# LudoMichaud/hlsjs-p2p-wrapper

Hardware: AMD Instinct MI355X
Metric: segments/sec + P2P offload ratio, 1080p 6 Mb/s HLS at 1/2/4/8 MI355X (higher is better)
Workload: dtype uint8

## Files before the change

hlsjs_p2p_wrapper_amd/agent/node.py:

```python
from __future__ import annotations

import contextlib
import logging
import os
import threading
import time
import zlib
from dataclasses import dataclass, field
from typing import Any, Dict, List, Optional, Tuple

import numpy as np
import torch

from ..net import http
from ..net.event_loop import get_event_loop
from ..ops import crc as _crc
from ..ops import segment as _seg
from ..ops._native import runtime as _rt
from ..parallel.comm import LocalComm, SwarmComm
from ..utils.trace import PhaseTimer, RequestTrace, TraceLog

log = logging.getLogger("hlsjs_p2p_wrapper_amd.node")

MAGIC = 0x48505032
HDR = 16
CHECK_WORD = 10
CDN_BOUND_BUSY = 0.6
ALIGN = 256
SLACK = 4096
PIN_DELAY_ROUNDS = 2


def swarm_id_for(content_id: str) -> int:
    return zlib.crc32(content_id.encode()) & 0x7FFFFFFF


_M32 = 0xFFFFFFFF


W_FORCE_CDN, W_NOT_STAGED, W_STAGING, W_PREFETCH, W_PY, W_CORRUPT = 1, 2, 4, 8, 16, 32
W_ON_DEV = 128
SRC_CDN, SRC_P2P, SRC_CACHE = 0, 1, 2
SOURCE_NAMES = ("cdn", "p2p", "cache")


class SwarmPeerLost(TimeoutError):
    """A swarm collective did not complete: a peer died, or stopped answering within the
    round / control deadline (``gpuSwarm.roundTimeoutMs`` / ``controlTimeoutMs``).  The
    message carries this rank's plan of the last round it posted."""


class Request:

    __slots__ = ("node", "key", "url", "headers", "callbacks", "agent", "aborted", "done", "t_submit", "token")

    def __init__(self, node: "SwarmNode", key: Tuple[int, int, int, int], url: str, headers: Dict[str, str],
                 callbacks: Any, agent: Any = None, aborted: bool = False, done: bool = False,
                 t_submit: float = 0.0) -> None:
        self.node = node
        self.key = key
        self.url = url
        self.headers = headers
        self.callbacks = callbacks
        self.agent = agent
        self.aborted = aborted
        self.done = done
        self.t_submit = t_submit
        self.token = None

    def abort(self) -> None:
        if not self.aborted:
            self.aborted = True
            if self.token is not None:
                self.node._abort_token(self.token)

    def __repr__(self) -> str:
        return f"Request(key={self.key}, url={self.url!r}, aborted={self.aborted}, done={self.done})"


class _WantX:

    __slots__ = ("url", "headers", "net", "src", "staged", "staging")

    def __init__(self, url: str, headers: Dict[str, str], net=None, src=None, staged: bool = True) -> None:
        self.url = url
        self.headers = headers
        self.net = net
        self.src = src
        self.staged = staged
        self.staging = False


@dataclass(eq=False)
class RoundHandle:
    round: int
    all_leaving: bool
    empty: bool = True
    ids: Any = None
    cdn: Any = None
    recv: Any = None
    failed: Any = None
    send_pins: Optional[np.ndarray] = None
    hold: List[np.ndarray] = field(default_factory=list)
    keep: List[Any] = field(default_factory=list)
    release: List[Any] = field(default_factory=list)
    sent_bytes: int = 0
    ev_cdn: Any = None
    dmas: int = 0
    ev_p2p: Any = None
    cdn_ms: float = 0.0
    p2p_ms: float = 0.0
    shaped_ms: float = 0.0
    ok_dev: Any = None
    ok_host: Any = None
    defer: Any = None
    expect_host: Any = None
    plan: Any = None
    t_post: float = 0.0
    done: Any = None
    n_wants: int = 0
    n_send: int = 0
    t0: float = 0.0
    completed: bool = False


class VerifyTicket:

    __slots__ = ("node", "eid", "expect", "token", "stamp", "done")

    def __init__(self, node: "SwarmNode", eid: int, expect: int, token: int) -> None:
        self.node = node
        self.eid = eid
        self.expect = expect
        self.token = token
        self.stamp = int(node._vround[eid])
        self.done = False

    def report(self, ok: bool) -> None:
        if not self.done:
            self.done = True
            node, e = self.node, self.eid
            if node._vflag[e] and node._vround[e] == self.stamp:
                node.verify_done(np.array([e], dtype=np.int64), np.array([bool(ok)]),
                                 np.array([self.token], dtype=np.int64))

    def __repr__(self) -> str:
        return f"VerifyTicket(eid={self.eid}, expect={self.expect:#010x}, done={self.done})"


class _EventPool:

    def __init__(self) -> None:
        self._free: Dict[bool, List[Any]] = {True: [], False: []}

    def get(self, timing: bool = False):
        free = self._free[timing]
        return free.pop() if free else torch.cuda.Event(enable_timing=timing)

    def put(self, timing: bool, *events) -> None:
        self._free[timing].extend(e for e in events if e is not None)


class SwarmNode:

    def __init__(self, comm: Optional[SwarmComm] = None, device: Any = "auto", cache_bytes: int = 1 << 30,
                 loop=None, cdn_dedup: bool = True, round_interval_ms: Optional[float] = None,
                 auto_tick: bool = True, max_wants_per_round: Optional[int] = None) -> None:
        self.comm = comm or LocalComm()
        self.rank = self.comm.rank
        self.world = self.comm.world_size
        self.ingest_crc = self.world > 1 or os.environ.get("HLSP2P_INGEST_CRC", "0") == "1"
        if device in (None, "auto"):
            device = torch.device("cuda", torch.cuda.current_device()) if torch.cuda.is_available() else "cpu"
        self.device = torch.device(device)
        self.is_cuda = self.device.type == "cuda"
        self.loop = loop or get_event_loop()
        self.rt = _rt()
        self.cache_bytes = int(cache_bytes)
        self.store = self.rt.SegmentStore(self.cache_bytes, ALIGN)
        self.directory = self.rt.Directory()
        self.arena = torch.empty(self.cache_bytes + SLACK, dtype=torch.uint8, device=self.device)
        self.stream = torch.cuda.Stream(self.device) if self.is_cuda else None
        self.copy_stream = (torch.cuda.Stream(self.device) if self.is_cuda and
                            os.environ.get("HLSP2P_COPY_STREAM", "1") != "0" else None)
        with self._on_node_stream():
            self.crc_dev = torch.zeros(self._crc_capacity(), dtype=torch.int32, device=self.device)
        self._events = _EventPool()
        self._clk = None
        self.online = True
        self._upload_default = True
        self._download_default = True
        self._sessions: Dict[Any, Tuple[bool, bool]] = {}
        self.cdn_dedup = cdn_dedup
        self.round = 0
        self.round_interval_ms = round_interval_ms
        self.round_timeout_s: Optional[float] = None
        self._last_posted: Optional[RoundHandle] = None
        self._exit_at = None
        fe = os.environ.get("HLSP2P_FAULT_EXIT")
        if fe:
            fr, _, fk = fe.partition(":")
            if int(fr) == self.rank:
                self._exit_at = int(fk)
        self.auto_tick = auto_tick
        self.max_wants_per_round = max_wants_per_round
        self.leaving = False
        self.closed = False
        self.failed: Optional[str] = None
        self.last_complete: Optional[float] = None
        self._wt = self.rt.WantTable()
        self._wx: Dict[int, _WantX] = {}
        self._tok_req: Dict[int, Request] = {}
        self._next_tok = -2
        self._bulk: Any = None
        self._bulk_hits: List[Tuple[np.ndarray, np.ndarray]] = []
        self._bulk_hits_scheduled = False
        self._locs: Dict[Tuple[str, Optional[str]], Tuple[int, int, int, int]] = {}
        self._locs_gen = -1
        self._loc_keep: Dict[int, torch.Tensor] = {}
        self._locator = self.rt.SegmentLocator()
        self._locator_gen = -1
        self._locator_origins: Dict[int, Any] = {}
        self._locator_skip: set = set()
        self._tick_scheduled = False
        self._timer = None
        self._pins: List[Tuple[int, np.ndarray]] = []
        self._inflight: Dict[int, RoundHandle] = {}
        self._local_hits: Dict[int, int] = {}
        self._delayed: Dict[int, Tuple[np.ndarray, np.ndarray]] = {}
        self._delayed_seq = 0
        self.pin_holders: List[Any] = []
        self.expect_holders: List[Any] = []
        self.audit_on = os.environ.get("HLSP2P_AUDIT", "0") == "1"
        self._agents: List[Any] = []
        self._prefetched: Dict[Tuple[int, int, int, int], str] = {}
        self._net_wants = False
        self.peer_online = np.ones(self.world, dtype=bool)
        self.stats = {"cdn": 0, "p2p": 0, "upload": 0, "cache": 0, "rounds": 0, "crc_failures": 0,
                      "segments": 0, "cdn_segments": 0, "p2p_segments": 0, "prefetched": 0,
                      "p2p_links": 0, "p2p_wire": 0, "p2p_rejected": 0, "p2p_rejected_segments": 0,
                      "cache_segments": 0}
        self.swarm_stats = {"cdn": 0, "p2p": 0, "upload": 0}
        self.last_round: Dict[str, Any] = {}
        self.corrupt_next_recv = 0
        self.misroute_next_send = 0
        self.divergence_check = self.world > 1 and os.environ.get("HLSP2P_DIVERGENCE_CHECK", "1") != "0"
        self._plan_digest = 0
        self._plan_round = 0
        self.p2p_from = np.zeros(self.world, dtype=np.int64)
        self.verify_deferred = False
        self.cdn_balance = os.environ.get("HLSP2P_CDN_BALANCE", "0") == "1"
        self._cdn_busy = 0.0
        self._cdn_num = self._cdn_den = 0.0
        self._cdn_t = None
        self._vflag = np.zeros(0, dtype=bool)
        self._vinfo = np.zeros((0, 10), dtype=np.int64)
        self._vround = np.zeros(0, dtype=np.int64)
        self._vexp = np.zeros(0, dtype=np.int64)
        self._vwait: Dict[int, List[np.ndarray]] = {}
        self.defer_inproc = False
        self._force_cdn_keys: set = set()
        self.link_kbps: Dict[int, float] = {}
        self.timer = PhaseTimer()
        self.trace: Optional[TraceLog] = None
        self.metrics_server: Any = None
        self._lock = threading.RLock()
        if self.world > 1 and auto_tick:
            self._timer = self.loop.set_interval(self._timer_tick, round_interval_ms or 10.0)

    def attach(self, agent: Any) -> None:
        self._agents.append(agent)

    def detach(self, agent: Any) -> None:
        if agent in self._agents:
            self._agents.remove(agent)
        self._sessions.pop(agent, None)
        gone = [t for t, r in self._tok_req.items() if r.agent is agent]
        for t in gone:
            self._tok_req.pop(t, None)
            self._wt.abort1(t)

    def set_session_flags(self, session: Any, download: bool, upload: bool) -> None:
        self._sessions[session] = (bool(download), bool(upload))

    def session_flags(self, session: Any) -> Tuple[bool, bool]:
        return self._sessions.get(session, (self._download_default, self._upload_default))

    @property
    def download_on(self) -> bool:
        if self._sessions:
            return any(d for d, _ in self._sessions.values())
        return self._download_default

    @download_on.setter
    def download_on(self, on: bool) -> None:
        self._download_default = bool(on)

    @property
    def upload_on(self) -> bool:
        if self._sessions:
            return any(u for _, u in self._sessions.values())
        return self._upload_default

    @upload_on.setter
    def upload_on(self, on: bool) -> None:
        self._upload_default = bool(on)

    @property
    def flags(self) -> int:
        f = 0
        if self.online:
            f |= self.rt.FLAG_ONLINE
        if self.upload_on:
            f |= self.rt.FLAG_UPLOAD
        if self.download_on:
            f |= self.rt.FLAG_DOWNLOAD
        if self.cdn_dedup:
            f |= self.rt.FLAG_CDN_DEDUP
        if self.cdn_balance and self._cdn_busy > CDN_BOUND_BUSY:
            f |= self.rt.FLAG_CDN_BOUND
        return f

    def pending(self) -> int:
        return len(self._wt)

    def _resolve(self, url: str, headers: Optional[Dict[str, str]]) -> Tuple[int, int, int, int, Optional[_WantX]]:
        rng_hdr = (headers.get("Range") or headers.get("range")) if headers else None
        gen = http.generation()
        if gen != self._locs_gen:
            self._locs.clear()
            self._locs_gen = gen
        ck = (url, rng_hdr)
        hit = self._locs.get(ck)
        if hit is not None:
            return hit[0], hit[1], hit[2], hit[3], None
        origin, path = http.resolve(url)
        if id(origin) not in self._locator_origins or self._locator_gen != http.generation():
            self._register_locator(origin)
        rng = http.parse_range(headers) if headers else None
        if getattr(origin, "staged_fetch", False):
            size = origin.staged_size(path, rng)
            self._net_wants = True
            x = _WantX(url, dict(headers or {}), net=(origin, path, rng), staged=size is not None)
            return int(size or 0), 0, 0, W_PY | (0 if size is not None else W_NOT_STAGED), x
        locate = getattr(origin, "locate", None)
        loc = locate(path, url, rng) if locate is not None else None
        if loc is None:
            size = origin.size(path, url, rng)
            return int(size or 0), 0, 0, W_PY, _WantX(url, dict(headers or {}), src=(origin, path, rng))
        data, off, n = loc
        base = data.data_ptr()
        flags = 0
        if data.is_cuda:
            flags |= W_ON_DEV
        elif base not in self._loc_keep and self.is_cuda and not data.is_pinned():
            raise RuntimeError("CDN origin buffers must be pinned host memory for the async H2D path")
        self._loc_keep.setdefault(base, data)
        corrupt = bool(getattr(origin, "_corrupt", None)) and origin.should_corrupt(path)
        if corrupt:
            flags |= W_CORRUPT
        res = (int(n), base + int(off), base, flags)
        if not corrupt and not getattr(origin, "_failures", None):
            if len(self._locs) > 1 << 16:
                self._locs.clear()
            self._locs[ck] = res
        return res[0], res[1], res[2], res[3], None

    def _register_locator(self, origin: Any) -> None:
        if http.generation() != self._locator_gen:
            self._locator.clear()
            self._locator_origins.clear()
            self._locator_skip.clear()
            self._locator_gen = http.generation()
        if id(origin) in self._locator_skip:
            return
        dirs_fn = getattr(origin, "segment_dirs", None)
        if dirs_fn is None:
            self._locator_skip.add(id(origin))
            return
        dirs = dirs_fn()
        if not dirs:
            return
        if any(not d[5].is_cuda and self.is_cuda and not d[5].is_pinned() for d in dirs):
            self._locator_skip.add(id(origin))
            return
        for d, prefix, suffix, lo, hi, data, offs, lens in dirs:
            base = data.data_ptr()
            self._loc_keep.setdefault(base, data)
            self._locator.add_dir(d, prefix, suffix, int(lo), int(hi), base, W_ON_DEV if data.is_cuda else 0,
                                  np.asarray(offs, dtype=np.int64), np.asarray(lens, dtype=np.int64))
        self._locator_origins[id(origin)] = origin

    def _locator_usable(self) -> bool:
        if not len(self._locator) or self._locator_gen != http.generation():
            return False
        for o in self._locator_origins.values():
            if getattr(o, "_failures", None) or getattr(o, "_corrupt", None):
                self._locator.clear()
                self._locator_origins.clear()
                return False
        return True

    def request(self, key: Tuple[int, int, int, int], url: str, headers: Optional[Dict[str, str]],
                callbacks: Any, agent: Any = None, view: Any = None) -> Request:
        k0, k1, k2, k3 = key
        k = (int(k0) & _M32, int(k1) & _M32, int(k2) & _M32, int(k3) & _M32)
        req = Request(self, k, url, dict(headers) if headers else {}, callbacks, agent, False, False,
                      self.loop.now())
        eid = self.store.lookup1(*k)
        if eid >= 0:
            self.store.pin(np.array([eid], dtype=np.int64))
            self._local_hits[eid] = self._local_hits.get(eid, 0) + 1
            self.loop.call_soon(self._serve_local, req, eid)
            return req
        if self._prefetched:
            self._prefetched.pop(k, None)
        wt = self._wt
        flags = 0
        if agent is not None and self._sessions and not self.session_flags(agent)[0]:
            flags = W_FORCE_CDN
        if self._force_cdn_keys and k in self._force_cdn_keys:
            self._force_cdn_keys.discard(k)
            flags |= W_FORCE_CDN
        size = ptr = base = 0
        x = None
        if wt.lookup1(*k) < 0:
            try:
                size, ptr, base, wf, x = self._resolve(url, req.headers)
            except http.HttpError as e:
                self.loop.call_soon(self._fail, req, e)
                return req
            flags |= wf
        tok = self._next_tok
        self._next_tok = tok - 1
        req.token = tok
        self._tok_req[tok] = req
        r = wt.add1(k[0], k[1], k[2], k[3], size, ptr, base, flags, tok)
        if r < 0 and x is not None:
            self._wx[-r - 1] = x
        self._schedule()
        return req

    def set_bulk_sink(self, sink: Any) -> None:
        self._bulk = sink

    def request_batch(self, keys: np.ndarray, urls: List[str], headers: Optional[List[Optional[Dict[str, str]]]],
                      tokens: np.ndarray, force_cdn: Optional[np.ndarray] = None) -> None:
        n = len(tokens)
        if n == 0:
            return
        keys = np.ascontiguousarray(np.asarray(keys, dtype=np.int64).reshape(n, 4) & _M32)
        tokens = np.ascontiguousarray(tokens, dtype=np.int64)
        eids = self.store.lookup(keys, False)
        hit = eids >= 0
        if hit.any():
            he = eids[hit]
            self.store.pin(he)
            self._bulk_hits.append((tokens[hit], he))
            if not self._bulk_hits_scheduled:
                self._bulk_hits_scheduled = True
                self.loop.call_soon(self._serve_bulk_hits)
            miss = np.flatnonzero(~hit)
            if not len(miss):
                return
        else:
            miss = None
        if self._vflag.any():
            miss = self._park_on_pending(keys, tokens, miss)
            if miss is not None and not len(miss):
                return
        idx = range(n) if miss is None else miss.tolist()
        m = n if miss is None else len(miss)
        sizes = np.zeros(m, dtype=np.int64)
        ptrs = np.zeros(m, dtype=np.int64)
        bases = np.zeros(m, dtype=np.int64)
        flags = np.zeros(m, dtype=np.int64)
        if force_cdn is not None:
            fc = np.asarray(force_cdn, dtype=bool)
            flags[:] = np.where(fc if miss is None else fc[miss], W_FORCE_CDN, 0)
        if self._force_cdn_keys:
            fk = self._force_cdn_keys
            for j, row in enumerate((keys if miss is None else keys[miss]).tolist()):
                t = tuple(row)
                if t in fk:
                    fk.discard(t)
                    flags[j] |= W_FORCE_CDN
        xs: Dict[int, _WantX] = {}
        bad: List[Tuple[int, int]] = []
        resolve = self._resolve
        done = None
        if self._locator_usable():
            sel_urls = urls if miss is None else [urls[i] for i in idx]
            s_, p_, b_, f_, done, found = self._locator.resolve(sel_urls if isinstance(sel_urls, list)
                                                                else list(sel_urls))
            if headers is not None:
                done &= np.fromiter((not h or ("Range" not in h and "range" not in h)
                                     for h in (headers if miss is None else [headers[i] for i in idx])),
                                    dtype=bool, count=m)
            sizes[done] = s_[done]
            ptrs[done] = p_[done]
            bases[done] = b_[done]
            flags[done] |= f_[done]
            if done.all():
                idx = ()
        for j, i in enumerate(idx):
            if done is not None and done[j]:
                continue
            try:
                sizes[j], ptrs[j], bases[j], wf, x = resolve(urls[i], headers[i] if headers is not None else None)
            except http.HttpError as e:
                bad.append((j, int(e.status or 0) or 500))
                continue
            flags[j] |= wf
            if x is not None:
                xs[j] = x
        sel_keys = keys if miss is None else keys[miss]
        sel_tok = tokens if miss is None else tokens[miss]
        if bad:
            bj = np.asarray([j for j, _ in bad], dtype=np.int64)
            self._fail_bulk(sel_tok[bj], np.asarray([s for _, s in bad], dtype=np.int64))
            keep = np.ones(m, dtype=bool)
            keep[bj] = False
            remap = np.cumsum(keep) - 1
            xs = {int(remap[j]): x for j, x in xs.items()}
            sel_keys, sel_tok = sel_keys[keep], sel_tok[keep]
            sizes, ptrs, bases, flags = sizes[keep], ptrs[keep], bases[keep], flags[keep]
        if self._prefetched:
            for kk in map(tuple, sel_keys.tolist()):
                self._prefetched.pop(kk, None)
        ids, created = self._wt.add(sel_keys, sizes, ptrs, bases, flags, sel_tok)
        for j, x in xs.items():
            if created[j]:
                self._wx[int(ids[j])] = x
        self._schedule()

    def abort_tokens(self, tokens: np.ndarray) -> int:
        return int(self._wt.abort(np.ascontiguousarray(tokens, dtype=np.int64)))

    def _abort_token(self, token: int) -> None:
        self._tok_req.pop(token, None)
        self._wt.abort1(token)

    def _stage(self, wid: int, x: _WantX) -> None:
        if x.staging or x.staged or x.net is None:
            return
        origin, path, rng = x.net
        x.staging = True
        self._wt.set(wid, -1, W_STAGING, 0)
        loop = self.loop
        loop.hold()

        def done(n, err):
            try:
                loop.call_soon_threadsafe(self._on_staged, wid, x, n, err)
            finally:
                loop.release()

        origin.stage(path, x.url, rng, x.headers, done)

    def _on_staged(self, wid: int, x: _WantX, n, err) -> None:
        x.staging = False
        alive = self._wx.get(wid) is x
        if err is not None:
            if alive:
                self._finish_failed(np.array([wid], dtype=np.int64), err)
            return
        x.staged = True
        if alive and self._wt.set(wid, int(n), 0, W_STAGING | W_NOT_STAGED):
            self._schedule()
        else:
            origin, path, rng = x.net
            origin.release(path, rng)

    def prefetch(self, key: Tuple[int, int, int, int], url: str, headers: Optional[Dict[str, str]] = None) -> bool:
        k = tuple(int(v) & _M32 for v in key)
        if self._wt.lookup1(*k) >= 0 or self.store.lookup1(*k) >= 0:
            return False
        try:
            size, ptr, base, wf, x = self._resolve(url, dict(headers or {}))
        except http.HttpError:
            return False
        r = self._wt.add1(k[0], k[1], k[2], k[3], size, ptr, base, wf | W_PREFETCH, self.rt.NO_TOKEN)
        if r < 0 and x is not None:
            self._wx[-r - 1] = x
        self.stats["prefetched"] += 1
        self._schedule()
        return True

    def _schedule(self) -> None:
        if self.world == 1 and self.auto_tick and not self._tick_scheduled:
            self._tick_scheduled = True
            self.loop.call_soon(self._local_tick)

    def _local_tick(self) -> None:
        self._tick_scheduled = False
        if len(self._wt):
            self.tick()

    def _timer_tick(self) -> None:
        if not self.closed:
            self.tick()

    def _serve_local(self, req: Request, eid: int) -> None:
        try:
            if req.aborted:
                return
            off, n = (int(x) for x in self.store.entries(np.array([eid], dtype=np.int64))[0][:2])
            src = self._prefetched.pop(req.key, None)
            if src is None:
                self.stats["cache"] += n
                self.stats["cache_segments"] += 1
            self._deliver_req(req, src or "cache", n, 0.0, 0.0, self.arena[off:off + n], -1, eid)
        finally:
            self.store.unpin(np.array([eid], dtype=np.int64))
            n = self._local_hits.get(eid, 0) - 1
            if n > 0:
                self._local_hits[eid] = n
            else:
                self._local_hits.pop(eid, None)

    def _park_on_pending(self, keys: np.ndarray, tokens: np.ndarray, miss: Optional[np.ndarray]) -> np.ndarray:
        rows = np.arange(len(tokens)) if miss is None else miss
        pe = self.store.lookup(np.ascontiguousarray(keys[rows]), True)
        park = pe >= 0
        park[park] = pe[park] < len(self._vflag)
        park[park] = self._vflag[pe[park]]
        if not park.any():
            return rows if miss is not None else None
        for e, t in zip(pe[park].tolist(), tokens[rows[park]].tolist()):
            self._vwait.setdefault(e, []).append(t)
        self.stats["parked"] = self.stats.get("parked", 0) + int(park.sum())
        return rows[~park]

    def _release_parked(self, e: int, ok: bool) -> None:
        toks = np.asarray(self._vwait.pop(e), dtype=np.int64)
        if ok:
            arr = np.array([e], dtype=np.int64)
            ids = np.repeat(arr, len(toks))
            self.store.pin(ids)
            self._bulk_hits.append((toks, ids))
            if not self._bulk_hits_scheduled:
                self._bulk_hits_scheduled = True
                self.loop.call_soon(self._serve_bulk_hits)
        else:
            self._retry_cdn(self._vinfo[e], toks)

    def _serve_bulk_hits(self) -> None:
        self._bulk_hits_scheduled = False
        hits, self._bulk_hits = self._bulk_hits, []
        for tok, eids in hits:
            try:
                ent = self.store.entries(eids)
                offs, lens = ent[:, 0].copy(), ent[:, 1].copy()
                self.stats["cache"] += int(lens.sum())
                self.stats["cache_segments"] += len(tok)
                z = np.zeros(len(tok), dtype=np.float64)
                self._deliver_cols(tok, np.full(len(tok), SRC_CACHE, dtype=np.int8), lens, z, z, offs, eids)
            finally:
                self.store.unpin(eids)

    def _fail(self, req: Request, err: Exception) -> None:
        if req.aborted or req.done:
            return
        req.done = True
        cb = req.callbacks
        on_error = cb.get("onError") if isinstance(cb, dict) else getattr(cb, "onError", None)
        if on_error is not None:
            on_error(err)

    def _fail_bulk(self, tokens: np.ndarray, status: np.ndarray) -> None:
        if self._bulk is not None and len(tokens):
            self._bulk.fail(tokens, status)

    def _finish_failed(self, wids: np.ndarray, err: http.HttpError) -> None:
        tok, _, _ = self._wt.finish(np.ascontiguousarray(wids, dtype=np.int64))
        for w in wids.tolist():
            x = self._wx.pop(w, None)
            if x is not None and x.net is not None and x.staged:
                x.net[0].release(x.net[1], x.net[2])
        if not len(tok):
            return
        bulk = tok >= 0
        if bulk.any():
            self._fail_bulk(tok[bulk], np.full(int(bulk.sum()), int(err.status or 0) or 500, dtype=np.int64))
        for t in tok[~bulk].tolist():
            req = self._tok_req.pop(t, None)
            if req is not None:
                self.loop.call_soon(self._fail, req, err)

    def _encode(self, rows: np.ndarray, adds: np.ndarray, rms: np.ndarray) -> np.ndarray:
        hdr = np.zeros(HDR, dtype=np.int64)
        hdr[0] = MAGIC
        hdr[1] = self.flags
        hdr[2] = len(rows)
        hdr[3] = len(adds)
        hdr[4] = len(rms)
        hdr[5] = 1 if self.leaving else 0
        hdr[6] = self.round
        hdr[7] = self.stats["cdn"]
        hdr[8] = self.stats["p2p"]
        hdr[9] = self.stats["upload"]
        hdr[CHECK_WORD] = self.directory.digest
        hdr[CHECK_WORD + 1] = self._plan_digest
        hdr[CHECK_WORD + 2] = self._plan_round
        return np.concatenate([hdr, rows.reshape(-1), adds.reshape(-1).astype(np.int64),
                               rms.reshape(-1).astype(np.int64)])

    CRC_TABLE_MAX = 1 << 20

    def _crc_capacity(self) -> int:
        return int(min(max(1024, self.cache_bytes // (8 << 10) + 1), self.CRC_TABLE_MAX))

    def _on_node_stream(self):
        return torch.cuda.stream(self.stream) if self.stream is not None else contextlib.nullcontext()

    def _grow_crc(self, n: int) -> None:
        old = self.crc_dev
        if n <= old.numel():
            return
        with self._on_node_stream():
            new = torch.zeros(max(n, 2 * old.numel()), dtype=torch.int32, device=self.device)
            new[:old.numel()] = old
        if old.is_cuda:
            old.record_stream(self.stream)
        self.crc_dev = new

    def tick(self) -> bool:
        with self._lock:
            h = self.launch_round()
            self.complete_round(h)
            return h.all_leaving

    def launch_round(self) -> RoundHandle:
        h = self._launch_round()
        if self.audit_on:
            from .audit import audit_node

            audit_node(self, "launch_round")
        return h

    def complete_round(self, h: RoundHandle) -> None:
        self._complete_round(h)
        if self.audit_on:
            from .audit import audit_node

            audit_node(self, "complete_round")

    def _launch_round(self) -> RoundHandle:
        rt = self.rt
        t0 = time.perf_counter()
        self.round += 1
        self.stats["rounds"] += 1
        if self._exit_at is not None and self.round >= self._exit_at:
            log.error("rank %d: injected crash at round %d (HLSP2P_FAULT_EXIT)", self.rank, self.round)
            os._exit(17)
        if self.verify_deferred and self.round % 8 == 0 and len(self._vflag):
            self._sweep_pending()
        if self._pins:
            keep = []
            for rel, ids in self._pins:
                if rel <= self.round:
                    self.store.unpin(ids)
                else:
                    keep.append((rel, ids))
            self._pins = keep
        for agent in self._agents:
            hook = getattr(agent, "before_round", None)
            if hook is not None:
                hook()
        cap = self.max_wants_per_round
        ids, rows, dropped, too_big, deferred = self._wt.select(self.store, self.directory,
                                                               -1 if cap is None else int(cap), self.round)
        if len(dropped) and self._wx:
            for w in dropped.tolist():
                x = self._wx.pop(w, None)
                if x is not None and x.net is not None and x.staged:
                    x.net[0].release(x.net[1], x.net[2])
        if len(too_big):
            self._finish_failed(too_big, http.HttpError(507, "", f"segment exceeds the {self.cache_bytes}-byte cache"))
        if deferred:
            self.stats["deferred"] = self.stats.get("deferred", 0) + int(deferred)
        if len(rows):
            need = int(np.maximum((rows[:, 4] + (ALIGN - 1)) // ALIGN * ALIGN, ALIGN).sum())
            self.store.retire_region(need)
            if not self.store.wrap_for(need):
                raise RuntimeError("segment cache cannot wrap for the round (pinned entries block eviction)")
            if self.audit_on:
                from .audit import check_region

                check_region(self, need)
        adds, rms = self.store.take_delta()
        try:
            parts = self.comm.allgather_control(self._encode(rows, adds, rms))
        except Exception as e:
            raise self._peer_lost("control all-gather", e) from e
        try:
            all_wants, flags, all_leaving, swarm_tot = rt.ingest_control(
                self.directory, parts, MAGIC, HDR, CHECK_WORD if self.divergence_check else -1)
        except rt.SwarmDivergence as e:
            self._diverged(str(e))
            raise
        self.peer_online = (flags & rt.FLAG_ONLINE) != 0
        self.swarm_stats = {"cdn": int(swarm_tot[0]), "p2p": int(swarm_tot[1]), "upload": int(swarm_tot[2])}
        h = RoundHandle(self.round, all_leaving, t0=t0)
        h.ids = ids
        self._inflight[h.round] = h
        t_ctrl = time.perf_counter()
        self.timer.add("control", t_ctrl - t0)
        if not len(all_wants):
            self._plan_digest, self._plan_round = 0, self.round
            return h
        h.empty = False
        me = self.rank
        cdn_bytes = np.fromiter((int(p[7]) for p in parts), dtype=np.int64, count=len(parts)) \
            if self.cdn_balance and self.world > 1 else None
        plan, any_p2p, self._plan_digest = rt.plan_round_for(self.directory, all_wants, flags, self.world, me,
                                                             cdn_bytes)
        self._plan_round = self.round
        h.n_wants = len(all_wants)
        cdn_rows = plan[(plan[:, 5] == -1) & (plan[:, 6] == me)]
        if self._net_wants and self._wx:
            for wid in plan[(plan[:, 5] == -2) & (plan[:, 6] == me), 7].tolist():
                x = self._wx.get(wid)
                if x is not None:
                    self._stage(wid, x)
        send_rows = plan[plan[:, 5] == me]
        recv_rows = plan[(plan[:, 6] == me) & (plan[:, 5] >= 0)]
        h.n_send = len(send_rows)
        h.plan = (send_rows, recv_rows)
        self._last_posted = h
        send_eids = np.full(len(send_rows), -1, dtype=np.int64)
        cached = send_rows[:, 8] == 0
        if cached.any():
            eids = self.store.lookup(np.ascontiguousarray(send_rows[cached, :4]), False)
            send_eids[cached] = eids
            valid = eids[eids >= 0]
            if len(valid):
                self.store.pin(valid)
                h.send_pins = valid
            if self.misroute_next_send > 0:
                self._misroute(send_rows, send_eids)
        t_cdn0 = time.perf_counter()
        self.timer.add("plan", t_cdn0 - t_ctrl)
        with (torch.cuda.stream(self.stream) if self.is_cuda else contextlib.nullcontext()):
            if len(cdn_rows):
                self._cdn_phase(h, cdn_rows)
                seeded = np.flatnonzero(~cached)
                if len(seeded) and h.cdn is not None:
                    send_eids[seeded] = self.store.lookup(np.ascontiguousarray(send_rows[seeded, :4]), False)
            t_p2p0 = time.perf_counter()
            self.timer.add("cdn_enqueue", t_p2p0 - t_cdn0)
            if any_p2p:
                self._p2p_phase(h, send_rows, recv_rows, send_eids)
            h.sent_bytes = int(send_rows[:, 4].sum()) if len(send_rows) else 0
            if self.is_cuda:
                h.done = self._events.get(True)
                h.done.record(self.stream)
        self.timer.add("p2p_enqueue", time.perf_counter() - t_p2p0)
        return h

    def _complete_round(self, h: RoundHandle) -> None:
        if h.completed:
            return
        h.completed = True
        self._inflight.pop(h.round, None)
        if h.empty:
            self.last_complete = time.monotonic()
            self.last_round = {"wants": 0, "ms": (time.perf_counter() - h.t0) * 1e3}
            if h.ids is not None and len(h.ids):
                self._wt.requeue(h.ids, False)
            return
        t0 = time.perf_counter()
        if h.done is not None and not h.done.query():
            self._wait_round(h)
            self._clock_sync(h.done, time.perf_counter())
            h.done = None
        t1 = time.perf_counter()
        self.timer.add("wait_device", t1 - t0)
        if h.ev_cdn is not None:
            h.cdn_ms = h.ev_cdn[0].elapsed_time(h.ev_cdn[1])
            self._events.put(True, *h.ev_cdn)
        if h.ev_p2p is not None:
            h.p2p_ms = h.ev_p2p[0].elapsed_time(h.ev_p2p[1])
            if self._clk is not None:
                ev, t_host = self._clk
                q = t_host + ev.elapsed_time(h.ev_p2p[0]) / 1e3 - h.t_post
                self.timer.add("exchange_queued", max(0.0, q))
                self.timer.add("exchange_queued_n", 1.0)
            self._events.put(True, *h.ev_p2p)
        if h.done is not None:
            self._events.put(True, h.done)
            h.done = None
        wt = self._wt
        recv = h.recv
        good = bad = None
        dgood = exp_good = None
        if recv is not None:
            ok = (h.ok_host.numpy() if isinstance(h.ok_host, torch.Tensor) else np.asarray(h.ok_host)).astype(bool)
            if ok.all():
                good = recv
            else:
                good = tuple(c[ok] for c in recv)
                bad = tuple(c[~ok] for c in recv)
            if h.defer is not None:
                dgood = h.defer[ok]
                eh = h.expect_host.numpy() if isinstance(h.expect_host, torch.Tensor) else np.asarray(h.expect_host)
                eh = eh.astype(np.int32) ^ _crc.key_digest(recv[5])
                exp_good = eh.astype(np.int64)[ok]
                if not dgood.any():
                    dgood = None
            commit = good[2] if dgood is None else good[2][~dgood]
            if len(commit):
                self.store.commit(commit)
            self._count_p2p(good[4], True)
            if bad is not None:
                self.store.drop(bad[2])
                self.stats["crc_failures"] += len(bad[0])
                self._count_p2p(bad[4], False)
        if h.send_pins is not None:
            self.store.unpin(h.send_pins)
        for x in h.release:
            origin, path, rng = x.net
            origin.release(path, rng)
        self.stats["upload"] += h.sent_bytes
        t2 = time.perf_counter()
        if h.cdn is not None and len(h.cdn[0]):
            wids, eids, offs, lens = h.cdn[0], h.cdn[1], h.cdn[2], h.cdn[3]
            self.stats["cdn"] += int(lens.sum())
            self.stats["cdn_segments"] += len(wids)
            tok, idx, pf = wt.finish(wids)
            self._after_finish(wids, pf, h.cdn[4], "cdn")
            cdn_ms = max(h.cdn_ms, h.shaped_ms)
            k = len(tok)
            if k:
                self._deliver_cols(tok, np.zeros(k, dtype=np.int8), lens[idx], np.full(k, cdn_ms),
                                   np.zeros(k), offs[idx], eids[idx], delay=h.shaped_ms)
        if good is not None and len(good[0]):
            wids, srcs, eids, offs, lens, keys = good
            winfo = wt.info(np.ascontiguousarray(wids[dgood])) if dgood is not None else None
            tok, idx, pf = wt.finish(wids)
            exp_tok = None
            if dgood is not None:
                tok, idx, exp_tok = self._settle_deferred(h, good, dgood, exp_good, tok, idx, winfo)
            self._after_finish(wids, pf, keys, "p2p")
            k = len(tok)
            if k:
                p2p_ms = np.full(len(wids), h.p2p_ms)
                delay = None
                if self.link_kbps:
                    delay = np.zeros(len(wids))
                    link_q: Dict[int, int] = {}
                    for i, (src, n) in enumerate(zip(srcs.tolist(), lens.tolist())):
                        kbps = self.link_kbps.get(src)
                        if kbps:
                            link_q[src] = link_q.get(src, 0) + n
                            delay[i] = link_q[src] * 8.0 / kbps
                            p2p_ms[i] = max(p2p_ms[i], delay[i])
                    delay = delay[idx]
                self._deliver_cols(tok, np.ones(k, dtype=np.int8), lens[idx], np.zeros(k), p2p_ms[idx], offs[idx],
                                   eids[idx], peers=srcs[idx], delay=delay, expect=exp_tok)
        if bad is not None and len(bad[0]):
            wt.requeue(bad[0], True)
        if h.ids is not None and len(h.ids):
            served = [a for a in (h.cdn[0] if h.cdn is not None else None,
                                  h.recv[0] if h.recv is not None else None, h.failed) if a is not None and len(a)]
            rest = np.setdiff1d(h.ids, np.concatenate(served), assume_unique=False) if served else h.ids
            if len(rest):
                wt.requeue(rest, False)
        for ids in h.hold:
            self.store.unpin(ids)
        h.hold = []
        self.timer.add("commit", t2 - t1)
        self.timer.add("deliver", time.perf_counter() - t2)
        self.timer.add("dev_cdn_ms", h.cdn_ms / 1e3)
        now = time.perf_counter()
        if self._cdn_t is not None:
            self._cdn_num += 0.2 * (h.cdn_ms / 1e3 - self._cdn_num)
            self._cdn_den += 0.2 * ((now - self._cdn_t) - self._cdn_den)
            self._cdn_busy = min(1.0, self._cdn_num / self._cdn_den) if self._cdn_den > 0 else 0.0
        self._cdn_t = now
        self.timer.add("dev_p2p_ms", h.p2p_ms / 1e3)
        self.last_complete = time.monotonic()
        self.last_round = {"wants": h.n_wants, "cdn": 0 if h.cdn is None else len(h.cdn[0]), "send": h.n_send,
                           "recv": 0 if h.recv is None else len(h.recv[0]), "cdn_ms": h.cdn_ms, "dmas": h.dmas,
                           "p2p_ms": h.p2p_ms, "ms": (time.perf_counter() - h.t0) * 1e3}
        if wt.waiting:
            self._schedule()

    def _after_finish(self, wids: np.ndarray, prefetch_only: np.ndarray, keys: np.ndarray, source: str) -> None:
        if self._wx:
            for w in wids.tolist():
                x = self._wx.pop(w, None)
                if x is not None and x.net is not None and x.staged and source == "p2p":
                    x.net[0].release(x.net[1], x.net[2])
        if prefetch_only.any():
            for i in np.flatnonzero(prefetch_only).tolist():
                self._prefetched[tuple(int(v) for v in keys[i])] = source

    def _clock_sync(self, ev, t_host: float) -> None:
        old = self._clk
        self._clk = (ev, t_host)
        if old is not None:
            self._events.put(True, old[0])

    ROUND_SPIN_S = 0.02

    def _wait_round(self, h: RoundHandle) -> None:
        ev = h.done
        spin_end = time.perf_counter() + self.ROUND_SPIN_S
        while time.perf_counter() < spin_end:
            if ev.query():
                return
        check = getattr(self.comm, "async_error", None)
        deadline = time.perf_counter() + self.round_deadline_s()
        while not ev.query():
            err = check() if check is not None else ""
            if err:
                self.failed = self.failed or f"round {h.round}: data plane error: {err}"
                raise RuntimeError(f"rank {self.rank}: swarm round {h.round} failed in the data plane: {err}")
            if time.perf_counter() > deadline:
                summary = self.plan_summary(h)
                log.error("rank %d: swarm round %d did not complete; this rank's plan: %s", self.rank, h.round,
                          summary)
                self._dump_plan(h)
                self.failed = self.failed or f"round {h.round} did not complete within {self.round_deadline_s():g} s"
                raise SwarmPeerLost(f"rank {self.rank}: swarm round {h.round} did not complete on the device "
                                    f"within {self.round_deadline_s():g} s (gpuSwarm.roundTimeoutMs); a peer may have "
                                    f"stopped.  Plan: {summary}")
            time.sleep(1e-3)

    ROUND_TIMEOUT_S = 60.0

    def round_deadline_s(self) -> float:
        if self.round_timeout_s is not None:
            return float(self.round_timeout_s)
        return float(os.environ.get("HLSP2P_ROUND_TIMEOUT", str(self.ROUND_TIMEOUT_S)))

    def _peer_lost(self, where: str, err: BaseException) -> "SwarmPeerLost":
        summary = self.plan_summary(self._last_posted) if self._last_posted is not None else {}
        log.error("rank %d: swarm %s failed in round %d: %s; last posted plan: %s", self.rank, where, self.round,
                  err, summary)
        self._diverged(f"{where} failed: {err}")
        return SwarmPeerLost(f"rank {self.rank}: swarm {where} failed in round {self.round} ({type(err).__name__}: "
                             f"{err}); a peer may have stopped.  Plan of round "
                             f"{summary.get('round', '-')}: {summary}")

    @staticmethod
    def plan_summary(h: RoundHandle) -> Dict[str, Any]:
        out: Dict[str, Any] = {"round": h.round, "send": {}, "recv": {}}
        if h.plan is None:
            return out
        for name, rows, col in (("send", h.plan[0], 6), ("recv", h.plan[1], 5)):
            if len(rows):
                peers, inv = np.unique(rows[:, col], return_inverse=True)
                nbytes = np.bincount(inv, weights=rows[:, 4])
                count = np.bincount(inv)
                out[name] = {int(p): [int(c), int(b)] for p, c, b in zip(peers, count, nbytes)}
        return out

    def _dump_plan(self, h: RoundHandle) -> None:
        d = os.environ.get("HLSP2P_PLAN_DUMP")
        if not d or h.plan is None:
            return
        try:
            os.makedirs(d, exist_ok=True)
            np.savez(os.path.join(d, f"plan.r{h.round}.rank{self.rank}.npz"), send=h.plan[0], recv=h.plan[1],
                     directory_digest=np.int64(self.directory.digest))
        except OSError as e:
            log.warning("rank %d: plan dump failed: %s", self.rank, e)

    def _diverged(self, what: str) -> None:
        if self.failed is None:
            self.failed = what
        log.error("rank %d: %s", self.rank, what)
        abort = getattr(self.comm, "abort", None)
        if abort is not None:
            try:
                abort()
            except Exception as e:
                log.warning("rank %d: communicator abort failed: %s", self.rank, e)

    def _views(self, offs: List[int], lens: List[int]) -> List[torch.Tensor]:
        if not len(offs):
            return []
        if self.is_cuda:
            from ..ops._native import device as _dev

            return _dev().arena_views(self.arena, np.asarray(offs, dtype=np.int64), np.asarray(lens, dtype=np.int64))
        arena = self.arena
        return [arena[o:o + n] for o, n in zip(offs, lens)]

    def _cdn_phase(self, h: RoundHandle, cdn_rows: np.ndarray) -> None:
        wids = np.ascontiguousarray(cdn_rows[:, 7])
        info = self._wt.info(wids)
        ptrs = info[:, 5].copy()
        bases = info[:, 6].copy()
        lens = info[:, 4].copy()
        wflags = info[:, 7]
        keep = info[:, 0] >= 0
        failed: List[int] = []
        slow = np.flatnonzero(keep & ((wflags & W_PY) != 0))
        for i in slow.tolist():
            wid = int(wids[i])
            x = self._wx.get(wid)
            try:
                if x is None:
                    raise http.HttpError(500, "", "want lost its origin state")
                if x.net is not None:
                    origin, path, rng = x.net
                    data, off, n, _ = origin.resource_range(path, rng)
                    h.release.append(x)
                    self._wx.pop(wid, None)
                    x.staged = False
                else:
                    origin, path, rng = x.src
                    data, off, n, _ = origin.resource(path)
                    if rng is not None:
                        s, e = rng
                        e = n - 1 if e is None else min(e, n - 1)
                        off, n = off + s, max(0, e - s + 1)
                    if origin.should_corrupt(path):
                        wflags[i] |= W_CORRUPT
            except http.HttpError as e:
                self._finish_failed(np.array([wid], dtype=np.int64), e)
                failed.append(wid)
                keep[i] = False
                continue
            base = data.data_ptr()
            if not data.is_cuda and self.is_cuda and base not in self._loc_keep and not data.is_pinned():
                raise RuntimeError("CDN origin buffers must be pinned host memory for the async H2D path")
            if data.is_cuda:
                wflags[i] |= W_ON_DEV
            h.keep.append(data)
            ptrs[i], bases[i], lens[i] = base + int(off), base, int(n)
        if failed:
            h.failed = np.asarray(failed, dtype=np.int64)
        if not keep.all():
            wids, ptrs, bases, lens, wflags = wids[keep], ptrs[keep], bases[keep], lens[keep], wflags[keep]
            keys = np.ascontiguousarray(info[keep, :4])
        else:
            keys = np.ascontiguousarray(info[:, :4])
        if not len(wids):
            return
        res = self.store.reserve_run(keys, lens, self.round)
        if res is None:
            raise RuntimeError("segment cache cannot make room (pinned entries block eviction)")
        _, eids, offs = res
        self.store.pin(eids)
        h.hold.append(eids)
        self._grow_crc(int(eids.max()) + 1)
        if self.is_cuda:
            on_dev = (wflags & W_ON_DEV) != 0
            if on_dev.any() and not on_dev.all():
                raise RuntimeError("CDN origin buffers of one round must all be pinned host or all HBM")
            start = self._events.get(True)
            end = self._events.get(True)
            cs = self.copy_stream
            with (torch.cuda.stream(cs) if cs is not None else contextlib.nullcontext()):
                start.record(cs if cs is not None else self.stream)
                from ..ops._native import device as _dev

                h.dmas = _dev().h2d_batch(self.arena, offs, ptrs, lens, bases, ALIGN, bool(on_dev[0]))
                end.record(cs if cs is not None else self.stream)
            if cs is not None:
                self.stream.wait_event(end)
            h.ev_cdn = (start, end)
        else:
            t = time.perf_counter()
            self.rt.host_copy_batch(self.arena.data_ptr(), self.arena.numel(), offs, ptrs, lens)
            h.cdn_ms = (time.perf_counter() - t) * 1e3
        corrupt = np.flatnonzero((wflags & W_CORRUPT) != 0)
        for i in corrupt.tolist():
            if lens[i]:
                self.arena[int(offs[i]) + int(lens[i]) // 2] ^= 0xFF
        if self.ingest_crc:
            _crc.crc32_batch(self.arena, offs, lens, scatter_to=self.crc_dev, scatter_idx=eids, keys=keys)
        self.store.commit(eids)
        total = int(lens.sum())
        h.shaped_ms = http.Shaper.transfer_ms(total)
        h.cdn = (wids, eids, offs, lens, keys)

    def _p2p_phase(self, h: RoundHandle, send_rows: np.ndarray, recv_rows: np.ndarray,
                   send_eids: np.ndarray) -> None:
        sends: List[Tuple[int, torch.Tensor]] = []
        recvs: List[Tuple[int, torch.Tensor]] = []
        dev = self.device
        t_prep = time.perf_counter()
        srun, gath, rrun, rid_a, roff_a = self.store.p2p_layout(
            np.ascontiguousarray(send_rows), np.ascontiguousarray(send_eids, dtype=np.int64),
            np.ascontiguousarray(recv_rows), self.round)
        spans_plane = getattr(self.comm, "exchange_spans", None) if self.is_cuda else None
        if spans_plane is not None and len(srun) and not (srun[:, 3] == 0).all():
            spans_plane = None
        trailer_all = trailers = None
        if len(send_rows):
            present_all = send_eids >= 0
            idx = _dev_index(np.where(present_all, send_eids, 0), dev)
            trailer_all = torch.index_select(self.crc_dev, 0, idx)
            if not present_all.all():
                trailer_all[torch.from_numpy(np.flatnonzero(~present_all)).to(dev)] = -1
            spans = self._views(srun[:, 4].tolist(), srun[:, 5].tolist()) \
                if spans_plane is None and len(srun) and (srun[:, 3] == 0).all() else None
            for k, (dst, a, b, mode, off, total) in enumerate(srun.tolist() if spans_plane is None else ()):
                if mode == 0:
                    buf = spans[k] if spans is not None else self.arena[off:off + total]
                else:
                    buf = torch.zeros(total, dtype=torch.uint8, device=dev)
                    g = gath[gath[:, 0] == k]
                    if len(g):
                        _seg.copy_segments(self.arena, buf, g[:, 1], g[:, 2], g[:, 3])
                sends.append((dst, buf))
                sends.append((dst, trailer_all[a:b]))
        if len(rrun):
            trailers = torch.empty(len(recv_rows), dtype=torch.int32, device=dev)
            if spans_plane is None:
                views = self._views(rrun[:, 3].tolist(), rrun[:, 4].tolist())
                for (src, a, b, _, _), view in zip(rrun.tolist(), views):
                    recvs.append((src, view))
                    recvs.append((src, trailers[a:b]))
            h.hold.append(rid_a)
            np.add.at(self.p2p_from, rrun[:, 0], np.add.reduceat(recv_rows[:, 4], rrun[:, 1]))
            self._grow_crc(int(rid_a.max()) + 1)
            h.recv = (np.ascontiguousarray(recv_rows[:, 7]), np.ascontiguousarray(recv_rows[:, 5]), rid_a, roff_a,
                      np.ascontiguousarray(recv_rows[:, 4]), np.ascontiguousarray(recv_rows[:, :4]))
        self.timer.add("p2p_prep", time.perf_counter() - t_prep)
        t = time.perf_counter()
        h.t_post = t
        if self.is_cuda:
            start = self._events.get(True)
            end = self._events.get(True)
            start.record(self.stream)
        try:
            if spans_plane is not None:
                spans_plane(*_span_columns(self.arena.data_ptr(), srun, trailer_all, rrun, trailers))
            else:
                self.comm.exchange(sends, recvs)
        except Exception as e:
            raise self._peer_lost("data-plane exchange", e) from e
        if self.is_cuda:
            end.record(self.stream)
            h.ev_p2p = (start, end)
        else:
            h.p2p_ms = (time.perf_counter() - t) * 1e3
        if h.recv is None:
            return
        if self.corrupt_next_recv > 0:
            self.corrupt_next_recv -= 1
            o, n = int(roff_a[0]), int(recv_rows[0, 4])
            if n:
                self.arena[o + n // 2] ^= 0x5A
        defer = None
        if self.verify_deferred:
            wf = self._wt.info(np.ascontiguousarray(recv_rows[:, 7]))[:, 7]
            d = (wf & (W_PY | W_PREFETCH)) == 0
            defer = d if d.any() else None
        if defer is None:
            _, ok = _crc.crc32_batch(self.arena, roff_a, recv_rows[:, 4], expect_dev=trailers,
                                     scatter_to=self.crc_dev, scatter_idx=rid_a, keys=recv_rows[:, :4])
        else:
            ok = self._defer_verify(h, defer, trailers, roff_a, recv_rows, rid_a)
        if isinstance(ok, np.ndarray):
            h.ok_host = ok
        elif self.is_cuda:
            h.ok_host = torch.empty(ok.numel(), dtype=torch.uint8, pin_memory=True)
            h.ok_host.copy_(ok, non_blocking=True)
        else:
            h.ok_host = ok
        self.stats["p2p_wire"] += int(recv_rows[:, 4].sum())
        self.stats["p2p_links"] += len(rrun)

    def _defer_verify(self, h: RoundHandle, defer: np.ndarray, trailers, roff_a: np.ndarray, recv_rows: np.ndarray,
                      rid_a: np.ndarray):
        dev = self.device
        nd, dd = np.flatnonzero(~defer), np.flatnonzero(defer)
        h.defer = defer
        if not len(nd):
            self.crc_dev.index_copy_(0, _dev_index(rid_a, dev), trailers)
            self._expect_to_host(h, trailers)
            return np.ones(len(recv_rows), dtype=np.uint8)
        if self.is_cuda:
            from ..ops.desc import pack_to_device

            ix = pack_to_device({"nd": nd, "dd": dd, "rd": np.ascontiguousarray(rid_a[dd])}, dev)
        else:
            ix = {"nd": torch.from_numpy(nd), "dd": torch.from_numpy(dd), "rd": torch.from_numpy(rid_a[dd])}
        ok = torch.ones(len(recv_rows), dtype=torch.uint8, device=dev)
        if len(nd):
            _, ok_nd = _crc.crc32_batch(self.arena, roff_a[nd], recv_rows[nd, 4],
                                        expect_dev=torch.index_select(trailers, 0, ix["nd"]),
                                        scatter_to=self.crc_dev, scatter_idx=rid_a[nd], keys=recv_rows[nd, :4])
            ok.index_copy_(0, ix["nd"], ok_nd)
        if len(dd):
            self.crc_dev.index_copy_(0, ix["rd"], torch.index_select(trailers, 0, ix["dd"]))
        self._expect_to_host(h, trailers)
        return ok

    def _expect_to_host(self, h: RoundHandle, trailers) -> None:
        if self.is_cuda:
            h.expect_host = torch.empty(trailers.numel(), dtype=torch.int32, pin_memory=True)
            h.expect_host.copy_(trailers, non_blocking=True)
        else:
            h.expect_host = trailers.clone()

    def _settle_deferred(self, h: RoundHandle, good: tuple, dgood: np.ndarray, exp_good: np.ndarray,
                         tok: np.ndarray, idx: np.ndarray, winfo: np.ndarray):
        wids, _, eids, offs, lens, _ = good
        n = len(wids)
        info = np.zeros((n, winfo.shape[1]), dtype=winfo.dtype)
        info[dgood] = winfo
        now = dgood & (np.bincount(idx, minlength=n) == 0)
        neg = tok < 0
        if neg.any() and not self.defer_inproc:
            now |= dgood & (np.bincount(idx[neg], minlength=n) > 0)
        keep = None
        if now.any():
            nr = np.flatnonzero(now)
            exp = (exp_good[nr] & _M32).tolist()
            if self.is_cuda:
                with self._on_node_stream():
                    _, okd = _crc.crc32_batch(self.arena, offs[nr], lens[nr], expect=exp)
                    ok_now = okd.cpu().numpy().astype(bool)
            else:
                ok_now = _crc.crc32_batch(self.arena, offs[nr], lens[nr], expect=exp)[1].numpy().astype(bool)
            if ok_now.any():
                self.store.commit(eids[nr[ok_now]])
            bad = nr[~ok_now]
            if len(bad):
                self.store.drop(eids[bad])
                self.stats["crc_failures"] += len(bad)
                self._reject_p2p(lens[bad])
                keep = np.ones(len(tok), dtype=bool)
                for r in bad.tolist():
                    sel = idx == r
                    self._retry_cdn(info[r], tok[sel])
                    keep &= ~sel
            dgood = dgood & ~now
        pend = np.flatnonzero(dgood)
        if len(pend):
            pe = eids[pend]
            self.store.pin(pe)
            self._vpend_add(pe, info[pend], exp_good[pend])
        exp_row = np.full(n, -1, dtype=np.int64)
        exp_row[pend] = exp_good[pend] & _M32
        if keep is not None:
            tok, idx = tok[keep], idx[keep]
        return tok, idx, exp_row[idx]

    def _misroute(self, send_rows: np.ndarray, send_eids: np.ndarray) -> None:
        ids, keys = self.store.resident()
        if not len(ids):
            return
        lens = self.store.entries(ids)[:, 1]
        for i in np.flatnonzero(send_eids >= 0).tolist():
            same = np.flatnonzero((lens == send_rows[i, 4]) & (keys != send_rows[i, :4]).any(axis=1))
            if len(same):
                send_eids[i] = ids[same[0]]
                self.misroute_next_send -= 1
                return

    def _count_p2p(self, lens: np.ndarray, passed: bool) -> None:
        n = len(lens)
        if not n:
            return
        b = int(np.asarray(lens, dtype=np.int64).sum())
        if passed:
            self.stats["p2p"] += b
            self.stats["p2p_segments"] += n
        else:
            self.stats["p2p_rejected"] += b
            self.stats["p2p_rejected_segments"] += n

    def _reject_p2p(self, lens: np.ndarray) -> None:
        n = len(lens)
        if not n:
            return
        b = int(np.asarray(lens, dtype=np.int64).sum())
        self.stats["p2p"] -= b
        self.stats["p2p_segments"] -= n
        self.stats["p2p_rejected"] += b
        self.stats["p2p_rejected_segments"] += n

    def _vpend_add(self, eids: np.ndarray, info: np.ndarray, expect: np.ndarray) -> None:
        need = int(eids.max()) + 1
        if need > len(self._vflag):
            cap = max(need, 2 * len(self._vflag), 1024)
            flag = np.zeros(cap, dtype=bool)
            flag[:len(self._vflag)] = self._vflag
            vinfo = np.zeros((cap, self._vinfo.shape[1]), dtype=np.int64)
            vinfo[:len(self._vinfo)] = self._vinfo
            vround = np.zeros(cap, dtype=np.int64)
            vround[:len(self._vround)] = self._vround
            vexp = np.zeros(cap, dtype=np.int64)
            vexp[:len(self._vexp)] = self._vexp
            self._vflag, self._vinfo, self._vround, self._vexp = flag, vinfo, vround, vexp
        self._vflag[eids] = True
        self._vinfo[eids] = info
        self._vround[eids] = self.round
        self._vexp[eids] = expect

    VERIFY_STALE_ROUNDS = 32

    def _sweep_pending(self) -> int:
        stale = np.flatnonzero(self._vflag & (self._vround < self.round - self.VERIFY_STALE_ROUNDS))
        if not len(stale):
            return 0
        ent = self.store.entries(stale)
        offs, lens = ent[:, 0].copy(), ent[:, 1].copy()
        exp = (self._vexp[stale] & _M32).tolist()
        if self.is_cuda:
            with self._on_node_stream():
                _, okd = _crc.crc32_batch(self.arena, offs, lens, expect=exp)
                ok = okd.cpu().numpy().astype(bool)
        else:
            ok = _crc.crc32_batch(self.arena, offs, lens, expect=exp)[1].numpy().astype(bool)
        self.verify_done(stale, ok, np.full(len(stale), self.rt.NO_TOKEN, dtype=np.int64))
        self.stats["verify_swept"] = self.stats.get("verify_swept", 0) + len(stale)
        return len(stale)

    def pending_verify(self) -> int:
        return int(self._vflag.sum())

    def _retry_cdn(self, info: np.ndarray, tokens: np.ndarray) -> None:
        tokens = np.ascontiguousarray(tokens, dtype=np.int64)
        if not len(tokens):
            return
        n = len(tokens)
        rep = np.repeat(info.reshape(1, -1), n, axis=0)
        self._wt.add(np.ascontiguousarray(rep[:, :4]), np.ascontiguousarray(rep[:, 4]), np.ascontiguousarray(rep[:, 5]),
                     np.ascontiguousarray(rep[:, 6]), np.ascontiguousarray(rep[:, 7] | W_FORCE_CDN), tokens)
        self._schedule()

    def invalidate(self, keys) -> int:
        keys = np.ascontiguousarray(np.asarray(keys, dtype=np.int64).reshape(-1, 4) & _M32)
        if not len(keys):
            return 0
        eids = self.store.lookup(keys, False)
        held = eids[eids >= 0]
        if len(held):
            self.store.detach(held)
        for row in keys.tolist():
            self._force_cdn_keys.add(tuple(row))
        self.stats["invalidated"] = self.stats.get("invalidated", 0) + len(held)
        return len(held)

    def verify_done(self, eids: np.ndarray, ok: np.ndarray, tokens: np.ndarray) -> int:
        eids = np.asarray(eids, dtype=np.int64)
        ok = np.asarray(ok, dtype=bool)
        tokens = np.asarray(tokens, dtype=np.int64)
        if not len(eids):
            return 0
        ue, inv = np.unique(eids, return_inverse=True)
        uok = np.ones(len(ue), dtype=bool)
        np.logical_and.at(uok, inv, ok)
        inside = ue < len(self._vflag)
        pend = np.zeros(len(ue), dtype=bool)
        pend[inside] = self._vflag[ue[inside]]
        good = ue[pend & uok]
        if len(good):
            self._vflag[good] = False
            self.store.commit(good)
            self.store.unpin(good)
            if self._vwait:
                for e in good.tolist():
                    if e in self._vwait:
                        self._release_parked(e, True)
        bad = np.flatnonzero(pend & ~uok)
        for k in bad.tolist():
            e = int(ue[k])
            self._vflag[e] = False
            arr = np.array([e], dtype=np.int64)
            self.store.detach(arr)
            self.store.unpin(arr)
            self.stats["crc_failures"] += 1
            self._reject_p2p(self._vinfo[e:e + 1, 4])
            toks = tokens[inv == k]
            self._retry_cdn(self._vinfo[e], toks[toks >= 0])
            if e in self._vwait:
                self._release_parked(e, False)
            if (toks <= -2).any():
                self._force_cdn_keys.add(tuple(int(v) & _M32 for v in self._vinfo[e][:4]))
        return len(bad)

    def _deliver_cols(self, tok: np.ndarray, src: np.ndarray, nbytes: np.ndarray, cdn_ms: np.ndarray,
                      p2p_ms: np.ndarray, offs: np.ndarray, eids: np.ndarray, peers: Optional[np.ndarray] = None,
                      delay: Any = None, expect: Optional[np.ndarray] = None) -> None:
        if delay is not None and not (np.isscalar(delay) and delay <= 0):
            d = np.broadcast_to(np.asarray(delay, dtype=np.float64), tok.shape)
            later = d > 0
            if later.any():
                li = np.flatnonzero(later)
                le = eids[li]
                le = le[le >= 0]
                if len(le):
                    self.store.pin(le)
                self._delayed_seq += 1
                self._delayed[self._delayed_seq] = (le, tok[li])
                self.loop.set_timeout(self._deliver_deferred, float(d[li].max()),
                                      (tok[li], src[li], nbytes[li], cdn_ms[li], p2p_ms[li], offs[li], eids[li],
                                       None if peers is None else peers[li], None,
                                       None if expect is None else expect[li]), le, self._delayed_seq)
                if later.all():
                    return
                ni = np.flatnonzero(~later)
                tok, src, nbytes, cdn_ms, p2p_ms, offs, eids = (tok[ni], src[ni], nbytes[ni], cdn_ms[ni], p2p_ms[ni],
                                                                offs[ni], eids[ni])
                peers = None if peers is None else peers[ni]
                expect = None if expect is None else expect[ni]
        pin = eids[eids >= 0]
        if len(pin):
            self.store.pin(pin)
            self._pins.append((self.round + PIN_DELAY_ROUNDS, pin))
        bulk = tok >= 0
        nb = int(bulk.sum())
        if nb:
            self.stats["segments"] += nb
            if self._bulk is not None:
                ex = {} if expect is None else {"expect": expect if nb == len(tok) else expect[bulk]}
                if nb == len(tok):
                    self._bulk.deliver(tok, src, nbytes, cdn_ms, p2p_ms, offs, eids, **ex)
                else:
                    self._bulk.deliver(tok[bulk], src[bulk], nbytes[bulk], cdn_ms[bulk], p2p_ms[bulk], offs[bulk],
                                       eids[bulk], **ex)
        if nb == len(tok):
            return
        obj = np.flatnonzero(~bulk)
        reqs = [self._tok_req.pop(t, None) for t in tok[obj].tolist()]
        live = [i for i, r in zip(obj.tolist(), reqs) if r is not None]
        if not live:
            return
        views = self._views(offs[live].tolist(), nbytes[live].tolist())
        for i, r, view in zip(live, [r for r in reqs if r is not None], views):
            if expect is not None and expect[i] >= 0:
                view.swarm_verify = VerifyTicket(self, int(eids[i]), int(expect[i]), r.token)
            self._deliver_req(r, SOURCE_NAMES[int(src[i])], int(nbytes[i]), float(cdn_ms[i]), float(p2p_ms[i]), view,
                              self.rank if peers is None else int(peers[i]), int(eids[i]), pin=False)

    def _deliver_deferred(self, cols, ids: np.ndarray, seq: int = 0) -> None:
        self._delayed.pop(seq, None)
        try:
            self._deliver_cols(*cols)
        finally:
            if len(ids):
                self.store.unpin(ids)

    def _deliver_req(self, req: Request, source: str, nbytes: int, cdn_ms: float, p2p_ms: float, data: Any,
                     peer: int, eid: int, pin: bool = True) -> None:
        if req.aborted or req.done:
            return
        if pin and eid >= 0:
            arr = np.array([eid], dtype=np.int64)
            self.store.pin(arr)
            self._pins.append((self.round + PIN_DELAY_ROUNDS, arr))
        req.done = True
        self.stats["segments"] += 1
        trace = self.trace
        if trace is not None:
            now = self.loop.now()
            xfer = p2p_ms if source == "p2p" else cdn_ms
            trace.add(RequestTrace(req.key, req.t_submit, max(req.t_submit, now - xfer), now, source, nbytes,
                                   peer if source == "p2p" else self.rank, self.round))
        if req.agent is not None:
            req.agent._account(source, nbytes)
        cb = req.callbacks
        if isinstance(cb, dict):
            on_progress, on_success = cb.get("onProgress"), cb.get("onSuccess")
        else:
            delivered = getattr(cb, "onDelivered", None)
            if delivered is not None:
                delivered(source, nbytes, cdn_ms, p2p_ms, data)
                return
            on_progress, on_success = getattr(cb, "onProgress", None), getattr(cb, "onSuccess", None)
        if on_progress is not None:
            p2p = source in ("p2p", "cache")
            on_progress({"cdnDownloaded": 0 if p2p else nbytes, "p2pDownloaded": nbytes if p2p else 0,
                         "cdnDuration": 0.0 if p2p else cdn_ms, "p2pDuration": p2p_ms if p2p else 0.0})
        if req.aborted:
            return
        if on_success is not None:
            on_success(data)

    def enable_trace(self, maxlen: int = 100_000) -> TraceLog:
        if self.trace is None:
            self.trace = TraceLog(maxlen)
        return self.trace

    def save_cache(self, path: str) -> Dict[str, int]:
        from .checkpoint import save_cache

        return save_cache(self, path)

    def load_cache(self, path: str) -> Dict[str, int]:
        from .checkpoint import load_cache

        return load_cache(self, path)

    def set_link_bandwidth(self, peer: int, kbps: Optional[float]) -> None:
        if kbps:
            self.link_kbps[int(peer)] = float(kbps)
        else:
            self.link_kbps.pop(int(peer), None)

    def set_online(self, online: bool) -> None:
        self.online = bool(online)

    def close(self, timeout_rounds: int = 100000) -> None:
        self.leaving = True
        if self._timer is not None:
            self._timer.cancel()
            self._timer = None
        try:
            if self.world > 1:
                for _ in range(timeout_rounds):
                    if self.tick():
                        break
        finally:
            self.closed = True
            if self.metrics_server is not None:
                srv, self.metrics_server = self.metrics_server, None
                srv.close()

    def swarm_offload_ratio(self) -> float:
        c, p = self.swarm_stats["cdn"], self.swarm_stats["p2p"]
        return p / (p + c) if (p + c) else 0.0


def _span_columns(arena_ptr: int, srun: np.ndarray, trailer_all, rrun: np.ndarray, trailers):
    def cols(runs, span_off, span_len, tr):
        n = len(runs)
        ptr = np.empty(2 * n, dtype=np.int64)
        nb = np.empty(2 * n, dtype=np.int64)
        peer = np.empty(2 * n, dtype=np.int64)
        if n:
            ptr[0::2] = arena_ptr + runs[:, span_off]
            nb[0::2] = runs[:, span_len]
            ptr[1::2] = tr.data_ptr() + 4 * runs[:, 1]
            nb[1::2] = 4 * (runs[:, 2] - runs[:, 1])
            peer[0::2] = peer[1::2] = runs[:, 0]
        return ptr, nb, peer

    sp, sb, sd = cols(srun, 4, 5, trailer_all)
    rp, rb, rs = cols(rrun, 3, 4, trailers)
    return sp, sb, sd, rp, rb, rs


def _dev_index(idx: np.ndarray, dev: torch.device) -> torch.Tensor:
    if dev.type == "cuda":
        from ..ops.desc import pack_to_device

        return pack_to_device({"i": np.ascontiguousarray(idx, dtype=np.int64)}, dev)["i"]
    return torch.from_numpy(np.ascontiguousarray(idx, dtype=np.int64))


_local = threading.local()


def current_node() -> Optional[SwarmNode]:
    return getattr(_local, "node", None)


def set_current_node(node: Optional[SwarmNode]) -> None:
    _local.node = node


def node_for_config(p2p_config: Any) -> SwarmNode:
    apply_network_config(p2p_config)
    node = current_node()
    if node is not None and not node.closed:
        return node
    cfg = {}
    if isinstance(p2p_config, dict):
        cfg = dict(p2p_config.get("gpuSwarm") or {})
    backend = cfg.get("backend", "auto")
    comm: SwarmComm
    if backend == "auto":
        import torch.distributed as dist

        backend = "dist" if (dist.is_available() and dist.is_initialized() and dist.get_world_size() > 1) else "local"
    if backend == "local":
        comm = LocalComm()
    elif backend == "thread":
        comm = cfg["hub"].comm(int(cfg["rank"]))
    elif backend == "dist":
        from ..parallel.comm import DistComm

        comm = DistComm()
    elif backend == "remote":
        from ..parallel.fleet import RemoteNode

        node = RemoteNode(cfg["conn"], world=int(cfg.get("world", 1)), rank=int(cfg.get("rank", 0)),
                          payload=bool(cfg.get("fleetPayload", False)))
        set_current_node(node)
        return node
    else:
        raise ValueError(f"unknown gpuSwarm backend {backend!r}")
    node = SwarmNode(comm, device=cfg.get("device", "auto"), cache_bytes=int(cfg.get("cacheBytes", 1 << 30)),
                     cdn_dedup=bool(cfg.get("cdnDedup", True)), round_interval_ms=cfg.get("roundIntervalMs"),
                     auto_tick=bool(cfg.get("autoTick", True)), max_wants_per_round=cfg.get("maxWantsPerRound"))
    if cfg.get("numaBind") and node.is_cuda:
        from ..utils.runtime import bind_to_gpu_numa

        bind_to_gpu_numa(node.device.index if node.device.index is not None else torch.cuda.current_device())
    if cfg.get("audit"):
        node.audit_on = True
    if cfg.get("roundTimeoutMs") is not None:
        node.round_timeout_s = float(cfg["roundTimeoutMs"]) / 1e3
    if cfg.get("controlTimeoutMs") is not None and hasattr(comm, "control_timeout_s"):
        comm.control_timeout_s = float(cfg["controlTimeoutMs"]) / 1e3
    if cfg.get("deferVerify"):
        node.verify_deferred = node.defer_inproc = True
    if cfg.get("trace"):
        node.enable_trace()
    for peer, kbps in (cfg.get("linkKbps") or {}).items():
        node.set_link_bandwidth(int(peer), kbps)
    if cfg.get("metricsPort") is not None:
        node.metrics_server = _start_metrics(node, cfg, backend)
    set_current_node(node)
    return node


def apply_network_config(p2p_config: Any) -> None:
    gs = p2p_config.get("gpuSwarm") if isinstance(p2p_config, dict) else None
    net = gs.get("network") if isinstance(gs, dict) else None
    if net and not http.network_enabled():
        http.enable_network(True, **(net if isinstance(net, dict) else {}))


def _start_metrics(node: SwarmNode, cfg: dict, backend: str) -> Any:
    from ..utils.metrics import MetricsServer

    port = int(cfg["metricsPort"])
    if port:
        local = os.environ.get("LOCAL_RANK") if backend == "dist" else None
        port += int(local) if local is not None else node.rank
    try:
        return MetricsServer(node, port=port, host=str(cfg.get("metricsHost", "127.0.0.1")))
    except OSError as e:
        log.warning("metrics endpoint disabled on rank %d: cannot bind port %d (%s)", node.rank, port, e)
        return None
```

hlsjs_p2p_wrapper_amd/ops/csrc/kernels/bindings.cpp:

```cpp
#include <c10/hip/HIPStream.h>
#include <hip/hip_runtime_api.h>
#include <torch/extension.h>
#include <pybind11/numpy.h>
#include <pybind11/stl.h>

#include <cstring>

namespace hlsp2p {
namespace dev {
int aes_chunk_blocks();
hipError_t launch_aes128_cbc_decrypt(const uint8_t*, uint8_t*, const int64_t*, const int64_t*, const int64_t*,
                                     const int64_t*, const uint32_t*, const uint32_t*, const uint32_t*,
                                     const uint8_t*, int64_t*, int, int64_t, int, hipStream_t, const int64_t*,
                                     const void*, uint32_t*, const int64_t*, void*);
hipError_t launch_crc32_batch(const uint8_t*, const int64_t*, const int64_t*, const int64_t*, const int64_t*,
                              const void*, const uint32_t*, uint32_t*, uint32_t*, const uint32_t*, uint8_t*,
                              const int64_t*, uint32_t*, int64_t, int, int64_t, int, bool, hipStream_t,
                              const int64_t*);
hipError_t launch_ts_demux(const uint8_t*, const int64_t*, const int64_t*, const int64_t*, int, int64_t, uint32_t*,
                           int64_t*, int32_t*, uint8_t*, const int64_t*, int64_t*, int64_t, int64_t*, hipStream_t,
                           const void*, const int64_t*);
hipError_t launch_segment_copy(const uint8_t*, uint8_t*, const int64_t*, const int64_t*, const int64_t*,
                               const int64_t*, int, int64_t, hipStream_t);
}
}

namespace {

using torch::Tensor;
namespace D = hlsp2p::dev;

void check(const Tensor& t, const char* name, c10::ScalarType dt, int64_t min_numel = 0) {
  TORCH_CHECK(t.is_cuda(), name, " must be a GPU tensor");
  TORCH_CHECK(t.is_contiguous(), name, " must be contiguous");
  TORCH_CHECK(t.scalar_type() == dt, name, " has dtype ", t.scalar_type(), ", expected ", dt);
  TORCH_CHECK(t.numel() >= min_numel, name, " too small: ", t.numel(), " < ", min_numel);
}

void same_device(const Tensor& a, const Tensor& b) {
  TORCH_CHECK(a.device() == b.device(), "tensors on different devices");
}

hipStream_t stream() { return c10::hip::getCurrentHIPStream().stream(); }

void ok(hipError_t e, const char* what) {
  TORCH_CHECK(e == hipSuccess, what, " launch failed: ", hipGetErrorString(e));
}

int num_cus(const Tensor& t) {
  static int cached[64] = {0};
  const int dev = t.get_device();
  if (dev >= 0 && dev < 64 && cached[dev]) return cached[dev];
  int n = 0;
  hipDeviceGetAttribute(&n, hipDeviceAttributeMultiprocessorCount, dev);
  if (n <= 0) n = 256;
  if (dev >= 0 && dev < 64) cached[dev] = n;
  return n;
}

template <typename T>
const T* cptr(const Tensor& t) { return reinterpret_cast<const T*>(t.data_ptr()); }
template <typename T>
T* mptr(const Tensor& t) { return reinterpret_cast<T*>(t.data_ptr()); }

void aes128_cbc_decrypt(Tensor src, Tensor dst, Tensor src_off, Tensor dst_off, Tensor blk_prefix,
                        Tensor chunk_prefix, Tensor drk, Tensor iv, Tensor td0, Tensor isb, Tensor out_len,
                        int64_t total_chunks) {
  const int64_t B = src_off.numel();
  check(src, "src", torch::kUInt8);
  check(dst, "dst", torch::kUInt8);
  check(src_off, "src_off", torch::kInt64);
  check(dst_off, "dst_off", torch::kInt64, B);
  check(blk_prefix, "blk_prefix", torch::kInt64, B + 1);
  check(chunk_prefix, "chunk_prefix", torch::kInt64, B + 1);
  check(drk, "drk", torch::kInt32, B * 44);
  check(iv, "iv", torch::kUInt8, B * 16);
  check(td0, "td0", torch::kInt32, 256);
  check(isb, "isb", torch::kUInt8, 256);
  check(out_len, "out_len", torch::kInt64, B);
  TORCH_CHECK(src.data_ptr() != dst.data_ptr(), "CBC decrypt cannot run in place");
  TORCH_CHECK((reinterpret_cast<uintptr_t>(src.data_ptr()) & 15) == 0 &&
                  (reinterpret_cast<uintptr_t>(dst.data_ptr()) & 15) == 0,
              "src/dst must be 16-byte aligned");
  same_device(src, dst);
  ok(D::launch_aes128_cbc_decrypt(cptr<uint8_t>(src), mptr<uint8_t>(dst), cptr<int64_t>(src_off),
                                  cptr<int64_t>(dst_off), cptr<int64_t>(blk_prefix), cptr<int64_t>(chunk_prefix),
                                  cptr<uint32_t>(drk), cptr<uint32_t>(iv), cptr<uint32_t>(td0), cptr<uint8_t>(isb),
                                  mptr<int64_t>(out_len), static_cast<int>(B), total_chunks, num_cus(src), stream(),
                                  nullptr, nullptr, nullptr, nullptr, nullptr),
     "aes128_cbc_decrypt");
}

void crc32_batch(Tensor buf, Tensor seg_off, Tensor seg_len, Tensor tile_prefix, Tensor res_off, Tensor wfrag,
                 Tensor tables, Tensor residues, Tensor crc_out, c10::optional<Tensor> expect,
                 c10::optional<Tensor> ok_out, int64_t total_tiles, c10::optional<Tensor> scatter_idx,
                 c10::optional<Tensor> scatter_out) {
  const int64_t B = seg_off.numel();
  check(buf, "buf", torch::kUInt8);
  check(seg_off, "seg_off", torch::kInt64);
  check(seg_len, "seg_len", torch::kInt64, B);
  check(tile_prefix, "tile_prefix", torch::kInt64, B + 1);
  check(res_off, "res_off", torch::kInt64, B);
  const bool fp4 = wfrag.scalar_type() == torch::kUInt8;
  check(wfrag, "wfrag", fp4 ? torch::kUInt8 : torch::kInt8, fp4 ? 32 * 64 * 16 : 64 * 64 * 16);
  check(tables, "tables", torch::kInt32, 48 * 1024);
  check(residues, "residues", torch::kInt32);
  check(crc_out, "crc_out", torch::kInt32, B);
  TORCH_CHECK((reinterpret_cast<uintptr_t>(buf.data_ptr()) & 15) == 0, "buf must be 16-byte aligned");
  const uint32_t* ex = nullptr;
  uint8_t* okp = nullptr;
  if (expect.has_value()) {
    check(*expect, "expect", torch::kInt32, B);
    ex = cptr<uint32_t>(*expect);
  }
  if (ok_out.has_value()) {
    check(*ok_out, "ok_out", torch::kUInt8, B);
    okp = mptr<uint8_t>(*ok_out);
  }
  const int64_t* sidx = nullptr;
  uint32_t* sout = nullptr;
  int64_t sn = 0;
  TORCH_CHECK(scatter_idx.has_value() == scatter_out.has_value(), "scatter_idx and scatter_out go together");
  if (scatter_out.has_value()) {
    check(*scatter_idx, "scatter_idx", torch::kInt64, B);
    check(*scatter_out, "scatter_out", torch::kInt32);
    sidx = cptr<int64_t>(*scatter_idx);
    sout = mptr<uint32_t>(*scatter_out);
    sn = scatter_out->numel();
  }
  ok(D::launch_crc32_batch(cptr<uint8_t>(buf), cptr<int64_t>(seg_off), cptr<int64_t>(seg_len),
                           cptr<int64_t>(tile_prefix), cptr<int64_t>(res_off), wfrag.data_ptr(),
                           cptr<uint32_t>(tables), mptr<uint32_t>(residues), mptr<uint32_t>(crc_out), ex, okp,
                           sidx, sout, sn, static_cast<int>(B), total_tiles, num_cus(buf), fp4, stream(), nullptr),
     "crc32_batch");
}

void ts_demux(Tensor buf, Tensor seg_off, Tensor seg_len, Tensor blk_prefix, int64_t total_blocks, Tensor meta,
              Tensor pts_dts, Tensor blk_sums, Tensor es, Tensor es_off, Tensor pes, int64_t max_pes, Tensor info) {
  const int64_t B = seg_off.numel();
  check(buf, "buf", torch::kUInt8);
  check(seg_off, "seg_off", torch::kInt64);
  check(seg_len, "seg_len", torch::kInt64, B);
  check(blk_prefix, "blk_prefix", torch::kInt64, B + 1);
  check(meta, "meta", torch::kInt32, total_blocks * 256);
  check(pts_dts, "pts_dts", torch::kInt64, total_blocks * 256 * 2);
  check(blk_sums, "aux", torch::kInt32, total_blocks * 12 + B * 7);
  check(es, "es", torch::kUInt8);
  check(es_off, "es_off", torch::kInt64, B);
  check(pes, "pes", torch::kInt64, B * 3 * max_pes * 3);
  check(info, "info", torch::kInt64, B * 24);
  TORCH_CHECK((reinterpret_cast<uintptr_t>(buf.data_ptr()) & 15) == 0, "buf must be 16-byte aligned");
  ok(D::launch_ts_demux(cptr<uint8_t>(buf), cptr<int64_t>(seg_off), cptr<int64_t>(seg_len),
                        cptr<int64_t>(blk_prefix), static_cast<int>(B), total_blocks, mptr<uint32_t>(meta),
                        mptr<int64_t>(pts_dts), mptr<int32_t>(blk_sums), mptr<uint8_t>(es), cptr<int64_t>(es_off),
                        mptr<int64_t>(pes), max_pes, mptr<int64_t>(info), stream(), nullptr, nullptr),
     "ts_demux");
}

void segment_copy(Tensor src, Tensor dst, Tensor src_off, Tensor dst_off, Tensor len, Tensor chunk_prefix,
                  int64_t total_chunks) {
  const int64_t n = src_off.numel();
  check(src, "src", torch::kUInt8);
  check(dst, "dst", torch::kUInt8);
  check(src_off, "src_off", torch::kInt64);
  check(dst_off, "dst_off", torch::kInt64, n);
  check(len, "len", torch::kInt64, n);
  check(chunk_prefix, "chunk_prefix", torch::kInt64, n + 1);
  ok(D::launch_segment_copy(cptr<uint8_t>(src), mptr<uint8_t>(dst), cptr<int64_t>(src_off), cptr<int64_t>(dst_off),
                            cptr<int64_t>(len), cptr<int64_t>(chunk_prefix), static_cast<int>(n), total_chunks,
                            stream()),
     "segment_copy");
}

int64_t device_cus(Tensor t) { return num_cus(t); }

int64_t h2d_batch(Tensor dst, pybind11::array_t<int64_t> dst_off, pybind11::array_t<int64_t> src_ptr,
                  pybind11::array_t<int64_t> len, pybind11::array_t<int64_t> src_alloc, int64_t max_gap,
                  bool device_src) {
  check(dst, "dst", torch::kUInt8);
  const int64_t n = dst_off.size();
  TORCH_CHECK(src_ptr.size() == n && len.size() == n && src_alloc.size() == n, "h2d_batch: argument sizes differ");
  const int64_t* o = dst_off.data();
  const int64_t* s = src_ptr.data();
  const int64_t* l = len.data();
  const int64_t* a = src_alloc.data();
  uint8_t* base = mptr<uint8_t>(dst);
  const int64_t cap = dst.numel();
  hipStream_t st = stream();
  int64_t issued = 0;
  int64_t i = 0;
  while (i < n) {
    TORCH_CHECK(o[i] >= 0 && l[i] >= 0 && o[i] + l[i] <= cap, "h2d_batch: destination out of bounds");
    if (l[i] == 0) {
      ++i;
      continue;
    }
    int64_t j = i;
    while (j + 1 < n && l[j + 1] > 0 && a[j + 1] == a[j]) {
      const int64_t ds = o[j + 1] - o[j], ss = s[j + 1] - s[j];
      if (ds != ss || ds < l[j] || ds - l[j] >= max_gap) break;
      TORCH_CHECK(o[j + 1] + l[j + 1] <= cap, "h2d_batch: destination out of bounds");
      ++j;
    }
    const int64_t bytes = o[j] + l[j] - o[i];
    ok(hipMemcpyAsync(base + o[i], reinterpret_cast<const void*>(s[i]), static_cast<size_t>(bytes),
                      device_src ? hipMemcpyDeviceToDevice : hipMemcpyHostToDevice, st),
       "hipMemcpyAsync");
    ++issued;
    i = j + 1;
  }
  return issued;
}

std::vector<Tensor> pack_h2d(const std::vector<pybind11::array>& arrays, int64_t device_index) {
  namespace py = pybind11;
  std::vector<py::array> arr;
  arr.reserve(arrays.size());
  std::vector<int64_t> offs;
  std::vector<c10::ScalarType> types;
  int64_t total = 0;
  for (const auto& a0 : arrays) {
    py::array a = py::array::ensure(a0, py::array::c_style);
    TORCH_CHECK(a, "pack_h2d: not an array");
    const auto dt = a.dtype();
    const char kind = dt.kind();
    const auto size = dt.itemsize();
    c10::ScalarType st;
    if ((kind == 'i' || kind == 'u') && size == 8) st = torch::kInt64;
    else if ((kind == 'i' || kind == 'u') && size == 4) st = torch::kInt32;
    else if (kind == 'u' && size == 1) st = torch::kUInt8;
    else if (kind == 'i' && size == 1) st = torch::kInt8;
    else if (kind == 'f' && size == 8) st = torch::kFloat64;
    else TORCH_CHECK(false, "pack_h2d: unsupported dtype");
    offs.push_back(total);
    types.push_back(st);
    total += (static_cast<int64_t>(a.nbytes()) + 15) & ~int64_t(15);
    arr.push_back(std::move(a));
  }
  if (total < 16) total = 16;
  Tensor host = torch::empty({total}, torch::TensorOptions().dtype(torch::kUInt8).pinned_memory(true));
  uint8_t* h = host.data_ptr<uint8_t>();
  for (size_t i = 0; i < arr.size(); ++i) std::memcpy(h + offs[i], arr[i].data(), arr[i].nbytes());
  Tensor dev = torch::empty({total}, torch::TensorOptions().dtype(torch::kUInt8).device(torch::kCUDA, device_index));
  dev.copy_(host, true);
  std::vector<Tensor> out;
  out.reserve(arr.size());
  for (size_t i = 0; i < arr.size(); ++i) {
    const int64_t nb = static_cast<int64_t>(arr[i].nbytes());
    out.push_back(dev.narrow(0, offs[i], nb).view(types[i]));
  }
  return out;
}

}

TORCH_LIBRARY(hlsp2p, m) {
  m.def("aes128_cbc_decrypt(Tensor src, Tensor(a!) dst, Tensor src_off, Tensor dst_off, Tensor blk_prefix, "
        "Tensor chunk_prefix, Tensor drk, Tensor iv, Tensor td0, Tensor isb, Tensor(b!) out_len, "
        "int total_chunks) -> ()");
  m.def("crc32_batch(Tensor buf, Tensor seg_off, Tensor seg_len, Tensor tile_prefix, Tensor res_off, Tensor wfrag, "
        "Tensor tables, Tensor(a!) residues, Tensor(b!) crc_out, Tensor? expect, Tensor(c!)? ok_out, "
        "int total_tiles, Tensor? scatter_idx, Tensor(d!)? scatter_out) -> ()");
  m.def("ts_demux(Tensor buf, Tensor seg_off, Tensor seg_len, Tensor blk_prefix, int total_blocks, "
        "Tensor(a!) meta, Tensor(b!) pts_dts, Tensor(c!) blk_sums, Tensor(d!) es, Tensor es_off, Tensor(e!) pes, "
        "int max_pes, Tensor(f!) info) -> ()");
  m.def("segment_copy(Tensor src, Tensor(a!) dst, Tensor src_off, Tensor dst_off, Tensor len, Tensor chunk_prefix, "
        "int total_chunks) -> ()");
}

TORCH_LIBRARY_IMPL(hlsp2p, CUDA, m) {
  m.impl("aes128_cbc_decrypt", &aes128_cbc_decrypt);
  m.impl("crc32_batch", &crc32_batch);
  m.impl("ts_demux", &ts_demux);
  m.impl("segment_copy", &segment_copy);
}

void register_rccl(pybind11::module& m);
void register_transmux(pybind11::module& m);
void register_ingest(pybind11::module& m);

PYBIND11_MODULE(TORCH_EXTENSION_NAME, m) {
  m.doc() = "hlsjs-p2p-wrapper-amd CDNA4 (gfx950) kernels";
  m.def("aes128_cbc_decrypt", &aes128_cbc_decrypt);
  m.def("aes_chunk_blocks", &D::aes_chunk_blocks);
  namespace py = pybind11;
  m.def("crc32_batch", &crc32_batch, py::arg("buf"), py::arg("seg_off"), py::arg("seg_len"), py::arg("tile_prefix"),
        py::arg("res_off"), py::arg("wfrag"), py::arg("tables"), py::arg("residues"), py::arg("crc_out"),
        py::arg("expect"), py::arg("ok_out"), py::arg("total_tiles"), py::arg("scatter_idx") = py::none(),
        py::arg("scatter_out") = py::none());
  m.def("ts_demux", &ts_demux);
  m.def("segment_copy", &segment_copy);
  m.def("device_cus", &device_cus);
  m.def("h2d_batch", &h2d_batch, pybind11::arg("dst"), pybind11::arg("dst_off"), pybind11::arg("src_ptr"),
        pybind11::arg("len"), pybind11::arg("src_alloc"), pybind11::arg("max_gap"),
        pybind11::arg("device_src") = false);
  m.def("pack_h2d", &pack_h2d);
  register_rccl(m);
  register_transmux(m);
  register_ingest(m);
  m.attr("ARCH") = "gfx950";
}
```

hlsjs_p2p_wrapper_amd/ops/csrc/kernels/ingest.cpp:

```cpp
#include <c10/hip/HIPStream.h>
#include <hip/hip_runtime_api.h>
#include <torch/extension.h>
#include <pybind11/numpy.h>
#include <pybind11/stl.h>

#include <cstring>
#include <vector>

namespace hlsp2p {
namespace dev {
hipError_t launch_crc32_batch(const uint8_t*, const int64_t*, const int64_t*, const int64_t*, const int64_t*,
                              const void*, const uint32_t*, uint32_t*, uint32_t*, const uint32_t*, uint8_t*,
                              const int64_t*, uint32_t*, int64_t, int, int64_t, int, bool, hipStream_t,
                              const int64_t*);
}
}

namespace {

namespace py = pybind11;
using torch::Tensor;
using I64 = py::array_t<int64_t, py::array::c_style | py::array::forcecast>;

int cus(int device) {
  static int cached[64] = {0};
  if (device >= 0 && device < 64 && cached[device]) return cached[device];
  int n = 0;
  hipDeviceGetAttribute(&n, hipDeviceAttributeMultiprocessorCount, device);
  if (n <= 0) n = 256;
  if (device >= 0 && device < 64) cached[device] = n;
  return n;
}

void put(std::vector<uint8_t>& blk, int64_t& off, const void* p, int64_t nbytes) {
  off = static_cast<int64_t>(blk.size());
  blk.resize(off + ((nbytes + 15) & ~int64_t(15)), 0);
  if (nbytes) std::memcpy(blk.data() + off, p, static_cast<size_t>(nbytes));
}

py::tuple crc32_launch(Tensor buf, I64 offs, I64 lens, Tensor wfrag, Tensor tables, c10::optional<Tensor> expect,
                       c10::optional<Tensor> scatter_to, c10::optional<I64> scatter_idx, c10::optional<I64> keys) {
  TORCH_CHECK_VALUE(buf.is_cuda() && buf.is_contiguous() && buf.scalar_type() == torch::kUInt8, "buf: contiguous GPU uint8");
  TORCH_CHECK_VALUE((reinterpret_cast<uintptr_t>(buf.data_ptr()) & 15) == 0, "buf must be 16-byte aligned");
  const int64_t B = offs.size();
  TORCH_CHECK_VALUE(lens.size() == B, "crc32_launch: offs / lens sizes differ");
  const bool fp4 = wfrag.scalar_type() == torch::kUInt8;
  TORCH_CHECK_VALUE(wfrag.is_cuda() && wfrag.numel() >= (fp4 ? 32 * 64 * 16 : 64 * 64 * 16), "wfrag");
  TORCH_CHECK_VALUE(tables.is_cuda() && tables.scalar_type() == torch::kInt32 && tables.numel() >= 48 * 1024, "tables");
  const int device = buf.get_device();
  const auto dev_opts = torch::TensorOptions().device(torch::kCUDA, device);
  if (B == 0)
    return py::make_tuple(torch::empty({0}, dev_opts.dtype(torch::kInt32)),
                          expect.has_value() ? py::cast(torch::empty({0}, dev_opts.dtype(torch::kUInt8))) : py::none());
  const int64_t* o = offs.data();
  const int64_t* n = lens.data();
  const int64_t cap = buf.numel();
  std::vector<int64_t> tile_prefix(B + 1, 0), res_off(B, 0);
  int64_t groups_total = 0;
  for (int64_t i = 0; i < B; ++i) {
    TORCH_CHECK_VALUE(o[i] >= 0 && n[i] >= 0 && o[i] + n[i] <= cap, "crc32_launch: range out of bounds");
    TORCH_CHECK_VALUE(o[i] % 16 == 0, "crc32_launch: offsets must be 16-byte aligned");
    const int64_t groups = (n[i] + 255) / 256;
    res_off[i] = groups_total;
    groups_total += groups;
    tile_prefix[i + 1] = tile_prefix[i] + (groups + 31) / 32;
  }
  const uint32_t* ex = nullptr;
  if (expect.has_value()) {
    TORCH_CHECK_VALUE(expect->is_cuda() && expect->scalar_type() == torch::kInt32 && expect->numel() >= B &&
                    expect->is_contiguous(),
                "expect: int32 GPU tensor of B values");
    ex = static_cast<const uint32_t*>(expect->data_ptr());
  }
  TORCH_CHECK_VALUE(scatter_to.has_value() == scatter_idx.has_value(), "scatter_to and scatter_idx go together");
  std::vector<uint8_t> blk;
  int64_t d_o, d_n, d_tp, d_ro, d_si = -1, d_k = -1;
  put(blk, d_o, o, B * 8);
  put(blk, d_n, n, B * 8);
  put(blk, d_tp, tile_prefix.data(), (B + 1) * 8);
  put(blk, d_ro, res_off.data(), B * 8);
  uint32_t* sout = nullptr;
  int64_t sn = 0;
  if (scatter_to.has_value()) {
    TORCH_CHECK_VALUE(scatter_to->is_cuda() && scatter_to->scalar_type() == torch::kInt32 && scatter_to->is_contiguous(),
                "scatter_to: int32 GPU tensor");
    const I64& si = *scatter_idx;
    TORCH_CHECK_VALUE(si.size() == B, "scatter_idx size");
    sn = scatter_to->numel();
    for (int64_t i = 0; i < B; ++i) TORCH_CHECK_VALUE(si.data()[i] >= 0 && si.data()[i] < sn, "scatter index out of range");
    put(blk, d_si, si.data(), B * 8);
    sout = static_cast<uint32_t*>(scatter_to->data_ptr());
  }
  if (keys.has_value()) {
    TORCH_CHECK_VALUE(keys->size() == 4 * B, "keys: int64[B, 4]");
    put(blk, d_k, keys->data(), B * 32);
  }
  const int64_t nbytes = static_cast<int64_t>(blk.size());
  Tensor host = torch::empty({nbytes}, torch::TensorOptions().dtype(torch::kUInt8).pinned_memory(true));
  std::memcpy(host.data_ptr<uint8_t>(), blk.data(), blk.size());
  const int64_t res_words = std::max<int64_t>(1, groups_total);
  const int64_t d_res = (nbytes + 255) / 256 * 256;
  const int64_t d_crc = d_res + (res_words * 4 + 255) / 256 * 256;
  const int64_t d_ok = d_crc + (B * 4 + 255) / 256 * 256;
  Tensor dblk = torch::empty({d_ok + B}, dev_opts.dtype(torch::kUInt8));
  dblk.narrow(0, 0, nbytes).copy_(host, true);
  uint8_t* base = dblk.data_ptr<uint8_t>();
  auto at = [&](int64_t off) { return reinterpret_cast<int64_t*>(base + off); };
  Tensor crc = dblk.narrow(0, d_crc, B * 4).view(torch::kInt32);
  Tensor ok = dblk.narrow(0, d_ok, B);
  hipStream_t st = c10::hip::getCurrentHIPStream(device).stream();
  const hipError_t e = hlsp2p::dev::launch_crc32_batch(
      static_cast<const uint8_t*>(buf.data_ptr()), at(d_o), at(d_n), at(d_tp), at(d_ro), wfrag.data_ptr(),
      static_cast<const uint32_t*>(tables.data_ptr()), reinterpret_cast<uint32_t*>(base + d_res),
      reinterpret_cast<uint32_t*>(base + d_crc), ex, ex ? base + d_ok : nullptr, d_si >= 0 ? at(d_si) : nullptr, sout,
      sn, static_cast<int>(B), tile_prefix[B], cus(device), fp4, st, d_k >= 0 ? at(d_k) : nullptr);
  TORCH_CHECK(e == hipSuccess, "crc32 launch failed: ", hipGetErrorString(e));
  return py::make_tuple(crc, ex ? py::cast(ok) : py::none());
}

std::vector<Tensor> arena_views(const Tensor& arena, I64 offs, I64 lens) {
  TORCH_CHECK_VALUE(arena.dim() == 1 && arena.is_contiguous(), "arena must be a contiguous 1-D tensor");
  const int64_t B = offs.size();
  TORCH_CHECK_VALUE(lens.size() == B, "arena_views: offs / lens sizes differ");
  const int64_t* o = offs.data();
  const int64_t* n = lens.data();
  const int64_t cap = arena.numel();
  std::vector<Tensor> out;
  out.reserve(static_cast<size_t>(B));
  for (int64_t i = 0; i < B; ++i) {
    TORCH_CHECK_VALUE(o[i] >= 0 && n[i] >= 0 && o[i] + n[i] <= cap, "arena_views: range out of bounds");
    out.push_back(arena.narrow(0, o[i], n[i]));
  }
  return out;
}

}

void register_ingest(py::module& m) {
  m.def("crc32_launch", &crc32_launch, py::arg("buf"), py::arg("offs"), py::arg("lens"), py::arg("wfrag"),
        py::arg("tables"), py::arg("expect") = py::none(), py::arg("scatter_to") = py::none(),
        py::arg("scatter_idx") = py::none(), py::arg("keys") = py::none());
  m.def("arena_views", &arena_views, py::arg("arena"), py::arg("offs"), py::arg("lens"));
}
```

hlsjs_p2p_wrapper_amd/ops/csrc/kernels/rccl_comm.cpp:

```cpp
#include <hip/hip_runtime_api.h>
#include <pybind11/numpy.h>
#include <pybind11/pybind11.h>
#include <rccl/rccl.h>

#include <cstring>
#include <memory>
#include <stdexcept>
#include <string>

namespace py = pybind11;

namespace {

void nccl_ok(ncclResult_t r, const char* what) {
  if (r != ncclSuccess) throw std::runtime_error(std::string("RCCL ") + what + ": " + ncclGetErrorString(r));
}

class RcclComm {
 public:
  RcclComm(const py::bytes& id_bytes, int world, int rank, int device) : world_(world), rank_(rank), device_(device) {
    const std::string id = id_bytes;
    if (id.size() != sizeof(ncclUniqueId)) throw std::invalid_argument("RcclComm: unique id must be 128 bytes");
    if (world < 1 || rank < 0 || rank >= world) throw std::invalid_argument("RcclComm: bad rank / world size");
    ncclUniqueId uid;
    std::memcpy(&uid, id.data(), sizeof(uid));
    ncclResult_t r;
    {
      py::gil_scoped_release nogil;
      if (hipSetDevice(device) != hipSuccess) throw std::runtime_error("RcclComm: hipSetDevice failed");
      r = ncclCommInitRank(&comm_, world, uid, rank);
    }
    nccl_ok(r, "ncclCommInitRank");
  }

  ~RcclComm() {
    if (comm_ != nullptr) ncclCommAbort(comm_);
  }

  void exchange(py::array_t<int64_t, py::array::c_style | py::array::forcecast> send_ptr,
                py::array_t<int64_t, py::array::c_style | py::array::forcecast> send_bytes,
                py::array_t<int64_t, py::array::c_style | py::array::forcecast> send_peer,
                py::array_t<int64_t, py::array::c_style | py::array::forcecast> recv_ptr,
                py::array_t<int64_t, py::array::c_style | py::array::forcecast> recv_bytes,
                py::array_t<int64_t, py::array::c_style | py::array::forcecast> recv_peer, int64_t stream) {
    if (comm_ == nullptr) throw std::runtime_error("RcclComm: communicator is closed");
    const int64_t ns = send_ptr.size(), nr = recv_ptr.size();
    if (send_bytes.size() != ns || send_peer.size() != ns || recv_bytes.size() != nr || recv_peer.size() != nr)
      throw std::invalid_argument("RcclComm.exchange: argument sizes differ");
    const int64_t *sp = send_ptr.data(), *sb = send_bytes.data(), *sd = send_peer.data();
    const int64_t *rp = recv_ptr.data(), *rb = recv_bytes.data(), *rs = recv_peer.data();
    for (int64_t i = 0; i < ns; ++i)
      if (sd[i] < 0 || sd[i] >= world_ || sb[i] < 0) throw std::invalid_argument("RcclComm.exchange: bad send");
    for (int64_t i = 0; i < nr; ++i)
      if (rs[i] < 0 || rs[i] >= world_ || rb[i] < 0) throw std::invalid_argument("RcclComm.exchange: bad recv");
    if (ns == 0 && nr == 0) return;
    hipStream_t st = reinterpret_cast<hipStream_t>(stream);
    ncclResult_t r = ncclSuccess;
    {
      py::gil_scoped_release nogil;
      r = ncclGroupStart();
      for (int64_t i = 0; r == ncclSuccess && i < ns; ++i)
        if (sb[i] > 0)
          r = ncclSend(reinterpret_cast<const void*>(sp[i]), static_cast<size_t>(sb[i]), ncclUint8,
                       static_cast<int>(sd[i]), comm_, st);
      for (int64_t i = 0; r == ncclSuccess && i < nr; ++i)
        if (rb[i] > 0)
          r = ncclRecv(reinterpret_cast<void*>(rp[i]), static_cast<size_t>(rb[i]), ncclUint8,
                       static_cast<int>(rs[i]), comm_, st);
      const ncclResult_t e = ncclGroupEnd();
      if (r == ncclSuccess) r = e;
    }
    nccl_ok(r, "send/recv group");
    ++rounds_;
  }

  std::string async_error() {
    if (comm_ == nullptr) return "";
    ncclResult_t a = ncclSuccess;
    nccl_ok(ncclCommGetAsyncError(comm_, &a), "ncclCommGetAsyncError");
    return a == ncclSuccess ? "" : ncclGetErrorString(a);
  }

  void close() {
    if (comm_ == nullptr) return;
    ncclComm_t c = comm_;
    comm_ = nullptr;
    py::gil_scoped_release nogil;
    ncclCommDestroy(c);
  }

  void abort() {
    if (comm_ == nullptr) return;
    ncclComm_t c = comm_;
    comm_ = nullptr;
    ncclCommAbort(c);
  }

  int comm_count() const {
    int n = 0;
    nccl_ok(ncclCommCount(live(), &n), "ncclCommCount");
    return n;
  }
  int comm_user_rank() const {
    int r = -1;
    nccl_ok(ncclCommUserRank(live(), &r), "ncclCommUserRank");
    return r;
  }
  int comm_device() const {
    int d = -1;
    nccl_ok(ncclCommCuDevice(live(), &d), "ncclCommCuDevice");
    return d;
  }

  bool closed() const { return comm_ == nullptr; }
  int world() const { return world_; }
  int rank() const { return rank_; }
  int device() const { return device_; }
  int64_t rounds() const { return rounds_; }

 private:
  ncclComm_t live() const {
    if (comm_ == nullptr) throw std::runtime_error("RcclComm: communicator is closed");
    return comm_;
  }
  ncclComm_t comm_ = nullptr;
  int world_, rank_, device_;
  int64_t rounds_ = 0;
};

py::bytes unique_id() {
  ncclUniqueId uid;
  nccl_ok(ncclGetUniqueId(&uid), "ncclGetUniqueId");
  return py::bytes(reinterpret_cast<const char*>(&uid), sizeof(uid));
}

std::string version() {
  int v = 0;
  nccl_ok(ncclGetVersion(&v), "ncclGetVersion");
  return std::to_string(v);
}

std::string pci_bus_id(int device) {
  char buf[64] = {0};
  if (hipDeviceGetPCIBusId(buf, sizeof(buf), device) != hipSuccess)
    throw std::runtime_error("hipDeviceGetPCIBusId failed for device " + std::to_string(device));
  return std::string(buf);
}

py::tuple link_type(int dev_a, int dev_b) {
  uint32_t type = 0, hops = 0;
  const hipError_t e = hipExtGetLinkTypeAndHopCount(dev_a, dev_b, &type, &hops);
  if (e != hipSuccess)
    throw std::runtime_error(std::string("hipExtGetLinkTypeAndHopCount: ") + hipGetErrorString(e));
  return py::make_tuple(type, hops);
}

}

void register_rccl(py::module& m) {
  m.def("rccl_unique_id", &unique_id, "ncclGetUniqueId (rank 0 of a new communicator)");
  m.def("rccl_version", &version);
  m.def("pci_bus_id", &pci_bus_id, py::arg("device"));
  m.def("link_type", &link_type, py::arg("dev_a"), py::arg("dev_b"));
  py::class_<RcclComm, std::shared_ptr<RcclComm>>(m, "RcclComm")
      .def(py::init<const py::bytes&, int, int, int>(), py::arg("unique_id"), py::arg("world"), py::arg("rank"),
           py::arg("device"))
      .def("exchange", &RcclComm::exchange, py::arg("send_ptr"), py::arg("send_bytes"), py::arg("send_peer"),
           py::arg("recv_ptr"), py::arg("recv_bytes"), py::arg("recv_peer"), py::arg("stream"))
      .def("async_error", &RcclComm::async_error)
      .def("close", &RcclComm::close)
      .def("abort", &RcclComm::abort)
      .def_property_readonly("closed", &RcclComm::closed)
      .def_property_readonly("world", &RcclComm::world)
      .def_property_readonly("rank", &RcclComm::rank)
      .def_property_readonly("device", &RcclComm::device)
      .def_property_readonly("rounds", &RcclComm::rounds)
      .def("comm_count", &RcclComm::comm_count)
      .def("comm_user_rank", &RcclComm::comm_user_rank)
      .def("comm_device", &RcclComm::comm_device);
}
```

hlsjs_p2p_wrapper_amd/ops/csrc/kernels/segment_ops.hip:

```cpp
#include "common.h"

namespace hlsp2p {
namespace dev {

constexpr int kCopyThreads = 256;
constexpr int64_t kCopyChunk = 64 * 1024;

__global__ __launch_bounds__(kCopyThreads) void segment_copy_kernel(
    const uint8_t* __restrict__ src, uint8_t* __restrict__ dst, const int64_t* __restrict__ src_off,
    const int64_t* __restrict__ dst_off, const int64_t* __restrict__ len, const int64_t* __restrict__ chunk_prefix,
    int ncopy) {
  const int64_t gchunk = blockIdx.x;
  const int c = find_seg_wave(chunk_prefix, ncopy, gchunk);
  const int64_t chunk = gchunk - chunk_prefix[c];
  const int64_t n = len[c];
  const int64_t beg = chunk * kCopyChunk;
  const int64_t end = beg + kCopyChunk < n ? beg + kCopyChunk : n;
  const uint8_t* s = src + src_off[c];
  uint8_t* d = dst + dst_off[c];
  const bool vec = ((reinterpret_cast<uintptr_t>(s) | reinterpret_cast<uintptr_t>(d)) & 15) == 0;
  int64_t i = beg;
  if (vec) {
    const int64_t vend = beg + ((end - beg) & ~int64_t(15));
    constexpr int kUnroll = 8;
    const int64_t last = vend - 16;
    for (int64_t o0 = beg + 16 * threadIdx.x; o0 < vend; o0 += 16 * kCopyThreads * kUnroll) {
      uint4 v[kUnroll];
#pragma unroll
      for (int u = 0; u < kUnroll; ++u) {
        const int64_t o = o0 + 16 * kCopyThreads * u;
        v[u] = *reinterpret_cast<const uint4*>(s + (o < last ? o : last));
      }
#pragma unroll
      for (int u = 0; u < kUnroll; ++u) {
        const int64_t o = o0 + 16 * kCopyThreads * u;
        *reinterpret_cast<uint4*>(d + (o < last ? o : last)) = v[u];
      }
    }
    i = vend;
  }
  for (int64_t o = i + threadIdx.x; o < end; o += kCopyThreads) d[o] = s[o];
}

hipError_t launch_segment_copy(const uint8_t* src, uint8_t* dst, const int64_t* src_off, const int64_t* dst_off,
                               const int64_t* len, const int64_t* chunk_prefix, int ncopy, int64_t total_chunks,
                               hipStream_t stream) {
  if (ncopy <= 0 || total_chunks <= 0) return hipSuccess;
  hipLaunchKernelGGL(segment_copy_kernel, dim3(static_cast<unsigned>(total_chunks)), dim3(kCopyThreads), 0, stream,
                     src, dst, src_off, dst_off, len, chunk_prefix, ncopy);
  return hipGetLastError();
}

}
}
```

hlsjs_p2p_wrapper_amd/parallel/comm.py:

```python
from __future__ import annotations

import atexit
import logging
import os
import secrets
import socket
import threading
from typing import Any, List, Optional, Sequence, Tuple

import numpy as np
import torch

log = logging.getLogger("hlsjs_p2p_wrapper_amd.comm")


RCCL_CU_RESERVE = 64


class SwarmComm:
    rank: int = 0
    world_size: int = 1

    def allgather_control(self, msg: np.ndarray) -> List[np.ndarray]:
        raise NotImplementedError

    def exchange(self, sends: Sequence[Tuple[int, torch.Tensor]], recvs: Sequence[Tuple[int, torch.Tensor]]) -> None:
        raise NotImplementedError

    def allreduce_sum(self, values: np.ndarray) -> np.ndarray:
        parts = self.allgather_control(np.asarray(values, dtype=np.int64))
        return np.sum(np.stack(parts), axis=0)

    def barrier(self) -> None:
        self.allgather_control(np.zeros(1, dtype=np.int64))

    def close(self) -> None:
        pass

    def abort(self) -> None:
        """Error path: stop the data plane without waiting on peers (no-op by default)."""


class LocalComm(SwarmComm):
    def __init__(self) -> None:
        self.rank = 0
        self.world_size = 1

    def allgather_control(self, msg: np.ndarray) -> List[np.ndarray]:
        return [np.asarray(msg, dtype=np.int64).copy()]

    def exchange(self, sends, recvs) -> None:
        if sends or recvs:
            raise RuntimeError("LocalComm has no peers")


class ThreadHub:

    def __init__(self, world_size: int, timeout: float = 120.0) -> None:
        self.world_size = world_size
        self.timeout = timeout
        self._barrier = threading.Barrier(world_size)
        self._slots: List[Optional[np.ndarray]] = [None] * world_size
        self._mail: dict = {}
        self._lock = threading.Lock()

    def comm(self, rank: int) -> "ThreadComm":
        return ThreadComm(self, rank)

    def wait(self) -> None:
        self._barrier.wait(self.timeout)

    def abort(self) -> None:
        self._barrier.abort()


class ThreadComm(SwarmComm):
    def __init__(self, hub: ThreadHub, rank: int) -> None:
        self.hub = hub
        self.rank = rank
        self.world_size = hub.world_size

    def allgather_control(self, msg: np.ndarray) -> List[np.ndarray]:
        hub = self.hub
        hub._slots[self.rank] = np.asarray(msg, dtype=np.int64).copy()
        hub.wait()
        out = [s.copy() for s in hub._slots]
        hub.wait()
        return out

    def exchange(self, sends, recvs) -> None:
        hub = self.hub
        with hub._lock:
            for dst, t in sends:
                hub._mail.setdefault((self.rank, dst), []).append(t)
        hub.wait()
        per_src: dict = {}
        for src, t in recvs:
            q = hub._mail.get((src, self.rank), [])
            i = per_src.get(src, 0)
            if i >= len(q):
                raise RuntimeError(f"rank {self.rank}: no matching send from {src}")
            s = q[i]
            per_src[src] = i + 1
            if s.numel() != t.numel():
                raise RuntimeError(f"rank {self.rank}: size mismatch from {src}: {s.numel()} != {t.numel()}")
            t.copy_(s.to(t.device), non_blocking=False)
        hub.wait()
        with hub._lock:
            for src in range(self.world_size):
                hub._mail.pop((src, self.rank), None)
        hub.wait()


class DistComm(SwarmComm):

    def __init__(self, control_group=None, data_group=None) -> None:
        import torch.distributed as dist

        if not dist.is_initialized():
            raise RuntimeError("torch.distributed is not initialized")
        self.dist = dist
        self.rank = dist.get_rank()
        self.world_size = dist.get_world_size()
        backend = dist.get_backend(data_group)
        plane = os.environ.get("HLSP2P_DATA_PLANE", "")
        if control_group is None:
            control_group = dist.new_group(backend="gloo") if backend != "gloo" else None
        self.control_group = control_group
        self.data_group = data_group
        self.data_backend = backend
        self._cap = 64
        self.control_timeout_s = float(os.environ.get("HLSP2P_CONTROL_TIMEOUT", str(self.CONTROL_TIMEOUT_S)))
        self.shm_slot_words = max(1024, int(os.environ.get("HLSP2P_SHM_SLOT_WORDS", str(self.SHM_SLOT_WORDS))))
        self.control_fallbacks = 0
        self._shm = self._open_shm_control() if self.world_size > 1 else None
        self.control_transport = "shm" if self._shm is not None else "gloo"
        self._rccl = None
        self.rehearsal = None
        self.rccl_log: Optional[str] = None
        self.peer_devices: dict = {}
        self._ipc: Optional[_IpcOutbox] = None
        if backend == "gloo" and plane == "ipc" and self.world_size > 1 and torch.cuda.is_available():
            self._ipc = _IpcOutbox.open(self)
        want_rccl = (backend == "nccl" or plane == "rccl") and torch.cuda.is_available()
        if want_rccl and os.environ.get("HLSP2P_NATIVE_RCCL", "1") != "0":
            self._rccl = self._open_native_rccl()
        if want_rccl and self._rccl is None:
            if backend != "nccl":
                self.data_group = dist.new_group(backend="nccl")
                self.data_backend = "nccl"
            t = torch.zeros(1, dtype=torch.int64, device=torch.device("cuda", torch.cuda.current_device()))
            dist.all_reduce(t, group=self.data_group)
            torch.cuda.synchronize()
        if self._rccl is not None and torch.cuda.is_available():
            try:
                from ..ops._native import device as _dev

                _dev().set_cu_reserve(int(os.environ.get("HLSP2P_RCCL_CU_RESERVE", str(RCCL_CU_RESERVE))))
            except Exception:
                pass
        self.data_transport = ("rccl-native" if self._rccl is not None else
                               "rccl-torch" if self.data_backend == "nccl" else
                               "hip-ipc" if self._ipc is not None else backend)

    def _open_native_rccl(self):
        dist, g = self.dist, self.control_group
        dev = None
        ok = True
        uid: List[object] = [None]
        gpu = None
        self.rehearsal = os.environ.get("HLSP2P_RCCL_REHEARSAL") or None
        if self.rehearsal is not None and self.data_backend != "gloo":
            raise RuntimeError("HLSP2P_RCCL_REHEARSAL needs a gloo default group with HLSP2P_DATA_PLANE=rccl "
                               "(bench.py's GPU launch), not an nccl one")
        if self.rehearsal == "socket":
            os.environ["NCCL_HOSTID"] = f"hlsp2p-rehearsal-{os.getpid()}-{self.rank}"
            os.environ.setdefault("NCCL_SOCKET_IFNAME", "lo")
            os.environ.setdefault("NCCL_IB_DISABLE", "1")
        elif self.rehearsal is not None:
            raise ValueError(f"unknown HLSP2P_RCCL_REHEARSAL {self.rehearsal!r} (expected 'socket')")
        from .wire import configure_rccl_log

        self.rccl_log = configure_rccl_log(self.rank)
        dev_index = torch.cuda.current_device()
        try:
            from ..ops._native import device as _dev

            dev = _dev()
            dev.rccl_version()
            gpu = dev.pci_bus_id(dev_index)
            if self.rank == 0:
                uid[0] = dev.rccl_unique_id()
        except Exception:
            ok = False
        flags: List[object] = [None] * self.world_size
        dist.all_gather_object(flags, (ok, _host_id(), gpu, self.rehearsal, dev_index), group=g)
        if not all(f[0] for f in flags):
            return None
        modes = [f[3] for f in flags]
        if len(set(modes)) > 1:
            raise RuntimeError(f"ranks disagree on HLSP2P_RCCL_REHEARSAL: {modes}")
        self.peer_devices = {r: (f[1], f[2], f[4]) for r, f in enumerate(flags)}
        seen: dict = {}
        for r, (_, host, bus, _, _) in enumerate(flags):
            if (host, bus) in seen and self.rehearsal is None:
                raise RuntimeError(f"RCCL data plane: ranks {seen[(host, bus)]} and {r} would share GPU {bus} on "
                                   f"host {host[0]}; RCCL needs one GPU per rank (rehearse ranks that share a "
                                   "GPU with --dist-backend ipc or gloo)")
            seen[(host, bus)] = r
        dist.broadcast_object_list(uid, src=0, group=g)
        comm, err = None, ""
        try:
            comm = dev.RcclComm(uid[0], self.world_size, self.rank, torch.cuda.current_device())
        except Exception as e:
            err = f"{type(e).__name__}: {e}"
        dist.all_gather_object(flags, err, group=g)
        if any(flags):
            if comm is not None:
                comm.abort()
            raise RuntimeError(f"native RCCL communicator init failed on some rank: {flags}")
        atexit.register(comm.abort)
        return comm

    SHM_SLOT_WORDS = 16384
    CONTROL_TIMEOUT_S = 300.0

    def _open_shm_control(self):
        if os.environ.get("HLSP2P_CONTROL", "auto") == "gloo":
            return None
        dist, g = self.dist, self.control_group
        hosts: List[object] = [None] * self.world_size
        dist.all_gather_object(hosts, _host_id(), group=g)
        if any(h != hosts[0] for h in hosts):
            return None
        from ..ops._native import runtime as _rt

        rt = _rt()
        name = [f"/hlsp2p_{os.getpid()}_{secrets.token_hex(6)}" if self.rank == 0 else None]
        dist.broadcast_object_list(name, src=0, group=g)
        shm, ok = None, True
        if self.rank == 0:
            try:
                shm = rt.ShmControl(name[0], 0, self.world_size, self.shm_slot_words, True)
            except Exception:
                ok = False
        flags: List[object] = [None] * self.world_size
        dist.all_gather_object(flags, ok, group=g)
        if self.rank != 0 and all(flags):
            try:
                shm = rt.ShmControl(name[0], self.rank, self.world_size, self.shm_slot_words, False)
            except Exception:
                ok = False
        dist.all_gather_object(flags, ok, group=g)
        if shm is not None and self.rank == 0:
            shm.unlink()
        return shm if all(flags) else None

    def allgather_control(self, msg: np.ndarray) -> List[np.ndarray]:
        if self._shm is not None:
            out = self._shm.allgather(np.ascontiguousarray(msg, dtype=np.int64).reshape(-1), self.control_timeout_s)
            if out is not None:
                return out
            self.control_fallbacks += 1
            if self.control_fallbacks == 1:
                log.warning("rank %d: a control message exceeded the %d-word shared-memory slot; this round's "
                            "all-gather fell back to gloo (raise HLSP2P_SHM_SLOT_WORDS; counted in "
                            "control_fallbacks)", self.rank, self.shm_slot_words)
        return self._allgather_gloo(msg)

    def _allgather_gloo(self, msg: np.ndarray) -> List[np.ndarray]:
        dist = self.dist
        msg = np.asarray(msg, dtype=np.int64).reshape(-1)
        cap = self._cap
        buf = torch.zeros(cap + 1, dtype=torch.int64)
        buf[0] = msg.size
        k = min(msg.size, cap)
        buf[1:1 + k] = torch.from_numpy(msg[:k])
        outs = [torch.empty(cap + 1, dtype=torch.int64) for _ in range(self.world_size)]
        dist.all_gather(outs, buf, group=self.control_group)
        sizes = [int(o[0]) for o in outs]
        mx = max(sizes)
        if mx <= cap:
            return [o[1:1 + n].numpy().copy() for o, n in zip(outs, sizes)]
        full = torch.zeros(mx, dtype=torch.int64)
        full[:msg.size] = torch.from_numpy(msg)
        outs = [torch.empty(mx, dtype=torch.int64) for _ in range(self.world_size)]
        dist.all_gather(outs, full, group=self.control_group)
        self._cap = max(cap, int(mx * 1.5) + 16)
        return [o[:n].numpy().copy() for o, n in zip(outs, sizes)]

    def exchange(self, sends, recvs) -> None:
        dist = self.dist
        if self._rccl is not None:
            self._exchange_native(sends, recvs)
            return
        if self._ipc is not None:
            self._ipc.exchange(sends, recvs)
            return
        if self.data_backend == "gloo" and any(t.is_cuda for _, t in list(sends) + list(recvs)):
            self._exchange_staged(sends, recvs)
            return
        ops = []
        for dst, t in sends:
            ops.append(dist.P2POp(dist.isend, t, dst, group=self.data_group))
        for src, t in recvs:
            ops.append(dist.P2POp(dist.irecv, t, src, group=self.data_group))
        if not ops:
            return
        reqs = dist.batch_isend_irecv(ops)
        for r in reqs:
            r.wait()

    @property
    def exchange_spans(self):
        if self._rccl is None:
            return None
        return self._exchange_spans

    def _exchange_spans(self, sp, sb, sd, rp, rb, rs) -> None:
        if len(sp) or len(rp):
            self._rccl.exchange(sp, sb, sd, rp, rb, rs, torch.cuda.current_stream().cuda_stream)

    def _exchange_native(self, sends, recvs) -> None:
        if not sends and not recvs:
            return
        ns, nr = len(sends), len(recvs)
        ptr = np.empty(ns + nr, dtype=np.int64)
        nbytes = np.empty(ns + nr, dtype=np.int64)
        peer = np.empty(ns + nr, dtype=np.int64)
        for i, (p, t) in enumerate(list(sends) + list(recvs)):
            if not (t.is_cuda and t.is_contiguous()):
                raise ValueError("native RCCL exchange needs contiguous GPU tensors")
            ptr[i] = t.data_ptr()
            nbytes[i] = t.numel() * t.element_size()
            peer[i] = p
        stream = torch.cuda.current_stream().cuda_stream
        self._rccl.exchange(ptr[:ns], nbytes[:ns], peer[:ns], ptr[ns:], nbytes[ns:], peer[ns:], stream)

    def async_error(self) -> str:
        if self._rccl is not None:
            return self._rccl.async_error()
        return ""

    def close(self) -> None:
        if self._rccl is not None:
            if torch.cuda.is_available():
                torch.cuda.synchronize()
            self._rccl.abort()
        if self._ipc is not None:
            self._ipc.close()

    def abort(self) -> None:
        if self._rccl is not None:
            self._rccl.abort()

    def topology(self) -> dict:
        out = {"transport": self.data_transport, "world": self.world_size, "rank": self.rank}
        if getattr(self, "rehearsal", None):
            out["rehearsal"] = self.rehearsal
        if self._rccl is not None and not self._rccl.closed:
            from ..ops._native import device as _dev

            out["rccl"] = {"count": int(self._rccl.comm_count()), "rank": int(self._rccl.comm_user_rank()),
                           "device": int(self._rccl.comm_device()), "rounds": int(self._rccl.rounds),
                           "version": _dev().rccl_version()}
            out["wire"] = self.wire()
        if self._ipc is not None:
            out["ipc_exchanges"] = int(self._ipc.exchanges)
        return out

    def wire(self) -> dict:
        from .wire import link_types, read_rccl_log, summarize

        rep = read_rccl_log(self.rccl_log, self.rank)
        out: dict = {"transport": summarize(rep, self.world_size)}
        if rep is not None:
            out.update(peers=rep["peers"], n_ranks=rep["n_ranks"], n_nodes=rep["n_nodes"],
                       local_ranks=rep["local_ranks"], connections=rep["connections"], log_bytes=rep["log_bytes"])
        else:
            out["peers"] = None
        me = self.peer_devices.get(self.rank)
        if me is not None:
            same_host = {r: d[2] for r, d in self.peer_devices.items() if r != self.rank and d[0] == me[0]}
            try:
                out["links"] = link_types(me[2], same_host) if same_host else {}
            except Exception as e:
                out["links"] = f"error: {e}"
        return out

    def _exchange_staged(self, sends, recvs) -> None:
        dist = self.dist
        torch.cuda.current_stream().synchronize()
        ops, staged = [], []
        for dst, t in sends:
            ops.append(dist.P2POp(dist.isend, t.detach().to("cpu"), dst, group=self.data_group))
        for src, t in recvs:
            h = torch.empty(t.numel(), dtype=t.dtype)
            staged.append((t, h))
            ops.append(dist.P2POp(dist.irecv, h, src, group=self.data_group))
        if ops:
            for r in dist.batch_isend_irecv(ops):
                r.wait()
        for t, h in staged:
            t.view(-1).copy_(h, non_blocking=False)

    def allreduce_sum(self, values: np.ndarray) -> np.ndarray:
        if self._shm is not None:
            return SwarmComm.allreduce_sum(self, values)
        t = torch.from_numpy(np.asarray(values, dtype=np.int64).copy())
        self.dist.all_reduce(t, group=self.control_group)
        return t.numpy()

    def barrier(self) -> None:
        if self._shm is not None:
            self._shm.barrier(self.control_timeout_s)
            return
        self.dist.barrier(group=self.control_group)


def _host_id() -> Tuple[str, str]:
    try:
        with open("/proc/sys/kernel/random/boot_id") as f:
            boot = f.read().strip()
    except OSError:
        boot = ""
    return socket.gethostname(), boot


def _as_bytes(t: torch.Tensor) -> torch.Tensor:
    if not t.is_contiguous():
        raise ValueError("IPC data plane needs contiguous tensors")
    return t.reshape(-1).view(torch.uint8)


def _outbox_slots(table: np.ndarray, me: int, align: int) -> List[Tuple[int, int]]:
    k = int(table[1])
    out, o = [], 0
    for d, n in zip(table[2:2 + 2 * k:2].tolist(), table[3:3 + 2 * k:2].tolist()):
        if d == me:
            out.append((o, n))
        o += (n + align - 1) // align * align
    return out


class _IpcOutbox:

    ALIGN = 256
    EVENT_RING = 8
    EVENT_RECORDS = 30

    def __init__(self, comm: "DistComm") -> None:
        self.comm = comm
        self.cap = 0
        self.buf: Optional[torch.Tensor] = None
        self.peers: List[torch.Tensor] = []
        self._pending = None
        self._ev: Optional[List[Any]] = None
        self._peer_ev: Optional[List[List[Any]]] = None
        self._ev_prev = None
        self._ev_gen_start = 0
        self.exchanges = 0

    @classmethod
    def open(cls, comm: "DistComm") -> Optional["_IpcOutbox"]:
        dist, g = comm.dist, comm.control_group
        hosts: List[object] = [None] * comm.world_size
        dist.all_gather_object(hosts, _host_id(), group=g)
        if any(h != hosts[0] for h in hosts):
            return None
        box = cls(comm)
        return box if box._share(int(os.environ.get("HLSP2P_IPC_OUTBOX_BYTES", str(1 << 30)))) else None

    def _share(self, cap: int) -> bool:
        from torch.multiprocessing.reductions import reduce_tensor

        comm = self.comm
        dist, g, me = comm.dist, comm.control_group, comm.rank
        cap = (max(cap, 1 << 20) + (1 << 20) - 1) // (1 << 20) * (1 << 20)
        handle = None
        try:
            self.buf = torch.empty(cap, dtype=torch.uint8, device=torch.device("cuda", torch.cuda.current_device()))
            torch.cuda.synchronize()
            handle = reduce_tensor(self.buf)
        except Exception:
            handle = None
        handles: List[object] = [None] * comm.world_size
        dist.all_gather_object(handles, handle, group=g)
        ok = all(h is not None for h in handles)
        if ok:
            try:
                self.peers = [self.buf if r == me else h[0](*h[1])
                              for r, h in enumerate(handles)]
            except Exception:
                ok = False
        flags: List[object] = [None] * comm.world_size
        dist.all_gather_object(flags, ok, group=g)
        if not all(flags):
            self.peers, self.buf = [], None
            return False
        self.cap = cap
        if os.environ.get("HLSP2P_IPC_EVENTS", "1") == "1":
            self._share_events()
        return True

    def _share_events(self) -> None:
        comm = self.comm
        dist, g, me = comm.dist, comm.control_group, comm.rank
        dev = torch.cuda.current_device()
        self._ev_prev = (self._ev, self._peer_ev)
        handle = None
        own: Optional[List[Any]] = None
        try:
            own = [torch.cuda.Event(enable_timing=False, interprocess=True) for _ in range(self.EVENT_RING)]
            for e in own:
                e.record()
            torch.cuda.synchronize()
            handle = [e.ipc_handle() for e in own]
        except Exception:
            handle = None
        handles: List[object] = [None] * comm.world_size
        dist.all_gather_object(handles, handle, group=g)
        evs: Optional[List[List[Any]]] = None
        if all(h is not None for h in handles):
            try:
                opened = torch.cuda.Event.from_ipc_handle
                evs = [own if r == me else [opened(dev, x) for x in h]
                       for r, h in enumerate(handles)]
            except Exception:
                evs = None
        flags: List[object] = [None] * comm.world_size
        dist.all_gather_object(flags, evs is not None, group=g)
        if all(flags):
            self._ev, self._peer_ev = own, evs
        else:
            self._ev, self._peer_ev = None, None
        self._ev_gen_start = self.exchanges

    def exchange(self, sends, recvs) -> None:
        comm = self.comm
        if self._pending is not None:
            self._pending.synchronize()
            self._pending = None
        A = self.ALIGN
        sizes = [int(t.numel()) * t.element_size() for _, t in sends]
        offs, pos = [], 0
        for n in sizes:
            offs.append(pos)
            pos += (n + A - 1) // A * A
        msg = np.empty(2 + 2 * len(sends), dtype=np.int64)
        msg[0], msg[1] = pos, len(sends)
        msg[2::2] = [d for d, _ in sends]
        msg[3::2] = sizes
        parts = comm.allgather_control(msg)
        need = max(int(p[0]) for p in parts)
        if need > self.cap:
            raise RuntimeError(f"IPC outbox of {self.cap} bytes cannot hold a round of {need} bytes "
                               "(raise HLSP2P_IPC_OUTBOX_BYTES)")
        stream = torch.cuda.current_stream()
        if self._peer_ev is not None and self.exchanges - self._ev_gen_start >= self.EVENT_RING * self.EVENT_RECORDS:
            self._share_events()
        slot = self.exchanges % self.EVENT_RING
        if sends:
            buf = self.buf
            for (_, t), o, n in zip(sends, offs, sizes):
                if n:
                    buf[o:o + n].copy_(_as_bytes(t), non_blocking=True)
            if self._peer_ev is not None:
                self._ev[slot].record(stream)
            else:
                stream.synchronize()
        comm.barrier()
        peer_ev = self._peer_ev
        me = comm.rank
        mine: dict = {}
        cursor: dict = {}
        for src, t in recvs:
            lst = mine.get(src)
            if lst is None:
                lst = mine[src] = _outbox_slots(parts[src], me, A)
                if peer_ev is not None and lst:
                    stream.wait_event(peer_ev[src][slot])
            i = cursor.get(src, 0)
            if i >= len(lst):
                raise RuntimeError(f"rank {me}: no matching send from {src}")
            cursor[src] = i + 1
            o, n = lst[i]
            dst = _as_bytes(t)
            if dst.numel() != n:
                raise RuntimeError(f"rank {me}: size mismatch from {src}: {n} != {dst.numel()}")
            if n:
                dst.copy_(self.peers[src][o:o + n], non_blocking=True)
        if recvs:
            ev = torch.cuda.Event()
            ev.record(stream)
            self._pending = ev
        self.exchanges += 1

    def close(self) -> None:
        if self._pending is not None:
            self._pending.synchronize()
            self._pending = None
        self.peers = []
        self.buf = None
```

Baseline: 18910.

## Post each round's CDN copies, ingest CRC and RCCL exchange through one native call

Adds a native round_post path that builds a single descriptor block, then on the stream launches the ingest CRC kernel, gathers CRC table entries for sends, posts the RCCL span exchange and scatters received CRCs. CDN copies go through a native round_copies call that merges adjacent ranges. The goal is to cut Python and per-call host overhead and the extra descriptor uploads in each round. It falls back to the old path for slow, corrupt, misroute or non-deferred-verify cases, which adds code complexity and more ways for the two paths to diverge.

```diff
diff --git a/hlsjs_p2p_wrapper_amd/agent/node.py b/hlsjs_p2p_wrapper_amd/agent/node.py
--- a/hlsjs_p2p_wrapper_amd/agent/node.py
+++ b/hlsjs_p2p_wrapper_amd/agent/node.py
@@ -249,6 +249,8 @@
         self._plan_round = 0
         self.p2p_from = np.zeros(self.world, dtype=np.int64)
         self.verify_deferred = False
+        self.round_post = os.environ.get("HLSP2P_ROUND_POST", "1") != "0"
+        self.native_posts = 0
         self.cdn_balance = os.environ.get("HLSP2P_CDN_BALANCE", "0") == "1"
         self._cdn_busy = 0.0
         self._cdn_num = self._cdn_den = 0.0
@@ -829,35 +831,45 @@
         h.n_send = len(send_rows)
         h.plan = (send_rows, recv_rows)
         self._last_posted = h
+        self._enqueue_round(h, cdn_rows, send_rows, recv_rows, any_p2p, t_ctrl)
+        return h
+
+    def _enqueue_round(self, h: RoundHandle, cdn_rows: np.ndarray, send_rows: np.ndarray, recv_rows: np.ndarray,
+                       any_p2p: bool, t_ctrl: float) -> None:
         send_eids = np.full(len(send_rows), -1, dtype=np.int64)
         cached = send_rows[:, 8] == 0
+        misroute = self.misroute_next_send > 0
+        post = _RoundPost() if (self.is_cuda and self.round_post and not misroute and self.corrupt_next_recv <= 0
+                                and getattr(self.comm, "exchange_spans", None) is not None) else None
         if cached.any():
             eids = self.store.lookup(np.ascontiguousarray(send_rows[cached, :4]), False)
             send_eids[cached] = eids
+            if misroute:
+                self._misroute(send_rows, send_eids)
+                eids = send_eids[cached]
             valid = eids[eids >= 0]
             if len(valid):
                 self.store.pin(valid)
                 h.send_pins = valid
-            if self.misroute_next_send > 0:
-                self._misroute(send_rows, send_eids)
         t_cdn0 = time.perf_counter()
         self.timer.add("plan", t_cdn0 - t_ctrl)
         with (torch.cuda.stream(self.stream) if self.is_cuda else contextlib.nullcontext()):
             if len(cdn_rows):
-                self._cdn_phase(h, cdn_rows)
+                post = self._cdn_phase(h, cdn_rows, post)
                 seeded = np.flatnonzero(~cached)
                 if len(seeded) and h.cdn is not None:
                     send_eids[seeded] = self.store.lookup(np.ascontiguousarray(send_rows[seeded, :4]), False)
             t_p2p0 = time.perf_counter()
             self.timer.add("cdn_enqueue", t_p2p0 - t_cdn0)
             if any_p2p:
-                self._p2p_phase(h, send_rows, recv_rows, send_eids)
+                self._p2p_phase(h, send_rows, recv_rows, send_eids, post)
+            elif post is not None:
+                self._post_native(h, post, False)
             h.sent_bytes = int(send_rows[:, 4].sum()) if len(send_rows) else 0
             if self.is_cuda:
                 h.done = self._events.get(True)
                 h.done.record(self.stream)
         self.timer.add("p2p_enqueue", time.perf_counter() - t_p2p0)
-        return h
 
     def _complete_round(self, h: RoundHandle) -> None:
         if h.completed:
@@ -1090,7 +1102,7 @@
         arena = self.arena
         return [arena[o:o + n] for o, n in zip(offs, lens)]
 
-    def _cdn_phase(self, h: RoundHandle, cdn_rows: np.ndarray) -> None:
+    def _cdn_phase(self, h: RoundHandle, cdn_rows: np.ndarray, post: "Optional[_RoundPost]" = None):
         wids = np.ascontiguousarray(cdn_rows[:, 7])
         info = self._wt.info(wids)
         ptrs = info[:, 5].copy()
@@ -1141,7 +1153,7 @@
         else:
             keys = np.ascontiguousarray(info[:, :4])
         if not len(wids):
-            return
+            return post
         res = self.store.reserve_run(keys, lens, self.round)
         if res is None:
             raise RuntimeError("segment cache cannot make room (pinned entries block eviction)")
@@ -1149,6 +1161,21 @@
         self.store.pin(eids)
         h.hold.append(eids)
         self._grow_crc(int(eids.max()) + 1)
+        if post is not None and (len(slow) or (wflags & W_CORRUPT).any()):
+            post = None
+        if post is not None:
+            self._cdn_copies_native(h, offs, ptrs, lens, bases, wflags)
+            post.cdn = (offs, lens, eids, keys)
+        else:
+            self._cdn_issue(h, offs, ptrs, lens, bases, wflags, eids, keys)
+        self.store.commit(eids)
+        total = int(lens.sum())
+        h.shaped_ms = http.Shaper.transfer_ms(total)
+        h.cdn = (wids, eids, offs, lens, keys)
+        return post
+
+    def _cdn_issue(self, h: RoundHandle, offs: np.ndarray, ptrs: np.ndarray, lens: np.ndarray, bases: np.ndarray,
+                   wflags: np.ndarray, eids: np.ndarray, keys: np.ndarray) -> None:
         if self.is_cuda:
             on_dev = (wflags & W_ON_DEV) != 0
             if on_dev.any() and not on_dev.all():
@@ -1175,13 +1202,9 @@
                 self.arena[int(offs[i]) + int(lens[i]) // 2] ^= 0xFF
         if self.ingest_crc:
             _crc.crc32_batch(self.arena, offs, lens, scatter_to=self.crc_dev, scatter_idx=eids, keys=keys)
-        self.store.commit(eids)
-        total = int(lens.sum())
-        h.shaped_ms = http.Shaper.transfer_ms(total)
-        h.cdn = (wids, eids, offs, lens, keys)
 
     def _p2p_phase(self, h: RoundHandle, send_rows: np.ndarray, recv_rows: np.ndarray,
-                   send_eids: np.ndarray) -> None:
+                   send_eids: np.ndarray, post: "Optional[_RoundPost]" = None) -> None:
         sends: List[Tuple[int, torch.Tensor]] = []
         recvs: List[Tuple[int, torch.Tensor]] = []
         dev = self.device
@@ -1193,6 +1216,17 @@
         if spans_plane is not None and len(srun) and not (srun[:, 3] == 0).all():
             spans_plane = None
         trailer_all = trailers = None
+        if post is not None:
+            ok = spans_plane is not None
+            if ok and len(rrun):
+                ok = self.verify_deferred and bool(
+                    ((self._wt.info(np.ascontiguousarray(recv_rows[:, 7]))[:, 7] & (W_PY | W_PREFETCH)) == 0).all())
+            if ok:
+                self._p2p_native(h, post, send_eids, recv_rows, srun, rrun, rid_a, roff_a, t_prep)
+                return
+            if post.cdn is not None and self.ingest_crc:
+                offs, lens, eids, keys = post.cdn
+                _crc.crc32_batch(self.arena, offs, lens, scatter_to=self.crc_dev, scatter_idx=eids, keys=keys)
         if len(send_rows):
             present_all = send_eids >= 0
             idx = _dev_index(np.where(present_all, send_eids, 0), dev)
@@ -1269,6 +1303,75 @@
         self.stats["p2p_wire"] += int(recv_rows[:, 4].sum())
         self.stats["p2p_links"] += len(rrun)
 
+    def _p2p_native(self, h: RoundHandle, post: "_RoundPost", send_eids: np.ndarray, recv_rows: np.ndarray,
+                    srun: np.ndarray, rrun: np.ndarray, rid_a: np.ndarray, roff_a: np.ndarray, t_prep: float) -> None:
+        n = len(recv_rows)
+        if len(rrun):
+            h.hold.append(rid_a)
+            np.add.at(self.p2p_from, rrun[:, 0], np.add.reduceat(recv_rows[:, 4], rrun[:, 1]))
+            self._grow_crc(int(rid_a.max()) + 1)
+            h.recv = (np.ascontiguousarray(recv_rows[:, 7]), np.ascontiguousarray(recv_rows[:, 5]), rid_a, roff_a,
+                      np.ascontiguousarray(recv_rows[:, 4]), np.ascontiguousarray(recv_rows[:, :4]))
+        self.timer.add("p2p_prep", time.perf_counter() - t_prep)
+        h.t_post = time.perf_counter()
+        post.p2p = (np.ascontiguousarray(send_eids, dtype=np.int64), srun, rrun, rid_a if len(rrun) else _NO_IDS)
+        self._post_native(h, post, True)
+        if h.recv is None:
+            return
+        h.defer = np.ones(n, dtype=bool)
+        h.ok_host = np.ones(n, dtype=np.uint8)
+        self.stats["p2p_wire"] += int(recv_rows[:, 4].sum())
+        self.stats["p2p_links"] += len(rrun)
+
+    def _timing_event(self):
+        ev = self._events.get(True)
+        if not ev.cuda_event:
+            ev.record(self.stream)
+        return ev
+
+    def _cdn_copies_native(self, h: RoundHandle, offs: np.ndarray, ptrs: np.ndarray, lens: np.ndarray,
+                           bases: np.ndarray, wflags: np.ndarray) -> None:
+        on_dev = (wflags & W_ON_DEV) != 0
+        if on_dev.any() and not on_dev.all():
+            raise RuntimeError("CDN origin buffers of one round must all be pinned host or all HBM")
+        from ..ops._native import device as _dev
+
+        cs = self.copy_stream
+        start, end = self._timing_event(), self._timing_event()
+        h.dmas = _dev().round_copies(self.arena, offs, ptrs, lens, bases, ALIGN, bool(on_dev[0]),
+                                     cs.cuda_stream if cs is not None else 0, start.cuda_event, end.cuda_event)
+        h.ev_cdn = (start, end)
+
+    def _post_native(self, h: RoundHandle, post: "_RoundPost", exchange: bool) -> None:
+        cdn, p2p = post.cdn, post.p2p
+        crc = cdn is not None and self.ingest_crc
+        if not crc and not exchange:
+            if cdn is not None:
+                self.native_posts += 1
+            return
+        from ..ops._native import device as _dev
+
+        dev = _dev()
+        z = _NO_IDS
+        offs = lens = eids = keys = z
+        w = tables = None
+        ep0 = ep1 = 0
+        if crc:
+            offs, lens, eids, keys = cdn
+            w, tables = _crc._device_consts(self.device, _crc.MFMA_VARIANT)
+        send_eids, srun, rrun, rid_a = p2p if p2p is not None else (z, z, z, z)
+        plane = None
+        if exchange:
+            h.ev_p2p = (self._timing_event(), self._timing_event())
+            ep0, ep1 = h.ev_p2p[0].cuda_event, h.ev_p2p[1].cuda_event
+            plane = getattr(self.comm, "rccl_native", None) or self.comm.exchange_spans
+        try:
+            h.expect_host = dev.round_post(self.arena, offs, lens, crc, eids, keys, w, tables, self.crc_dev,
+                                           send_eids, srun, rrun, rid_a, plane, exchange, ep0, ep1)
+        except dev.ExchangeError as e:
+            raise self._peer_lost("data-plane exchange", e) from e
+        self.native_posts += 1
+
     def _defer_verify(self, h: RoundHandle, defer: np.ndarray, trailers, roff_a: np.ndarray, recv_rows: np.ndarray,
                       rid_a: np.ndarray):
         dev = self.device
@@ -1624,6 +1727,18 @@
         return p / (p + c) if (p + c) else 0.0
 
 
+_NO_IDS = np.zeros(0, dtype=np.int64)
+
+
+class _RoundPost:
+
+    __slots__ = ("cdn", "p2p")
+
+    def __init__(self) -> None:
+        self.cdn = None
+        self.p2p = None
+
+
 def _span_columns(arena_ptr: int, srun: np.ndarray, trailer_all, rrun: np.ndarray, trailers):
     def cols(runs, span_off, span_len, tr):
         n = len(runs)
diff --git a/hlsjs_p2p_wrapper_amd/ops/csrc/kernels/bindings.cpp b/hlsjs_p2p_wrapper_amd/ops/csrc/kernels/bindings.cpp
--- a/hlsjs_p2p_wrapper_amd/ops/csrc/kernels/bindings.cpp
+++ b/hlsjs_p2p_wrapper_amd/ops/csrc/kernels/bindings.cpp
@@ -5,6 +5,8 @@
 #include <pybind11/stl.h>
 
 #include <cstring>
+
+#include "round_desc.h"
 
 namespace hlsp2p {
 namespace dev {
@@ -186,30 +188,7 @@
   const int64_t* a = src_alloc.data();
   uint8_t* base = mptr<uint8_t>(dst);
   const int64_t cap = dst.numel();
-  hipStream_t st = stream();
-  int64_t issued = 0;
-  int64_t i = 0;
-  while (i < n) {
-    TORCH_CHECK(o[i] >= 0 && l[i] >= 0 && o[i] + l[i] <= cap, "h2d_batch: destination out of bounds");
-    if (l[i] == 0) {
-      ++i;
-      continue;
-    }
-    int64_t j = i;
-    while (j + 1 < n && l[j + 1] > 0 && a[j + 1] == a[j]) {
-      const int64_t ds = o[j + 1] - o[j], ss = s[j + 1] - s[j];
-      if (ds != ss || ds < l[j] || ds - l[j] >= max_gap) break;
-      TORCH_CHECK(o[j + 1] + l[j + 1] <= cap, "h2d_batch: destination out of bounds");
-      ++j;
-    }
-    const int64_t bytes = o[j] + l[j] - o[i];
-    ok(hipMemcpyAsync(base + o[i], reinterpret_cast<const void*>(s[i]), static_cast<size_t>(bytes),
-                      device_src ? hipMemcpyDeviceToDevice : hipMemcpyHostToDevice, st),
-       "hipMemcpyAsync");
-    ++issued;
-    i = j + 1;
-  }
-  return issued;
+  return hlsp2p::host::issue_merged_copies(base, cap, o, s, l, a, n, max_gap, device_src, stream());
 }
 
 std::vector<Tensor> pack_h2d(const std::vector<pybind11::array>& arrays, int64_t device_index) {
@@ -278,6 +257,7 @@
 void register_rccl(pybind11::module& m);
 void register_transmux(pybind11::module& m);
 void register_ingest(pybind11::module& m);
+void register_round_post(pybind11::module& m);
 
 PYBIND11_MODULE(TORCH_EXTENSION_NAME, m) {
   m.doc() = "hlsjs-p2p-wrapper-amd CDNA4 (gfx950) kernels";
@@ -298,5 +278,6 @@
   register_rccl(m);
   register_transmux(m);
   register_ingest(m);
+  register_round_post(m);
   m.attr("ARCH") = "gfx950";
 }
diff --git a/hlsjs_p2p_wrapper_amd/ops/csrc/kernels/ingest.cpp b/hlsjs_p2p_wrapper_amd/ops/csrc/kernels/ingest.cpp
--- a/hlsjs_p2p_wrapper_amd/ops/csrc/kernels/ingest.cpp
+++ b/hlsjs_p2p_wrapper_amd/ops/csrc/kernels/ingest.cpp
@@ -6,6 +6,8 @@
 
 #include <cstring>
 #include <vector>
+
+#include "round_desc.h"
 
 namespace hlsp2p {
 namespace dev {
@@ -32,12 +34,6 @@
   return n;
 }
 
-void put(std::vector<uint8_t>& blk, int64_t& off, const void* p, int64_t nbytes) {
-  off = static_cast<int64_t>(blk.size());
-  blk.resize(off + ((nbytes + 15) & ~int64_t(15)), 0);
-  if (nbytes) std::memcpy(blk.data() + off, p, static_cast<size_t>(nbytes));
-}
-
 py::tuple crc32_launch(Tensor buf, I64 offs, I64 lens, Tensor wfrag, Tensor tables, c10::optional<Tensor> expect,
                        c10::optional<Tensor> scatter_to, c10::optional<I64> scatter_idx, c10::optional<I64> keys) {
   TORCH_CHECK_VALUE(buf.is_cuda() && buf.is_contiguous() && buf.scalar_type() == torch::kUInt8, "buf: contiguous GPU uint8");
@@ -55,16 +51,6 @@
   const int64_t* o = offs.data();
   const int64_t* n = lens.data();
   const int64_t cap = buf.numel();
-  std::vector<int64_t> tile_prefix(B + 1, 0), res_off(B, 0);
-  int64_t groups_total = 0;
-  for (int64_t i = 0; i < B; ++i) {
-    TORCH_CHECK_VALUE(o[i] >= 0 && n[i] >= 0 && o[i] + n[i] <= cap, "crc32_launch: range out of bounds");
-    TORCH_CHECK_VALUE(o[i] % 16 == 0, "crc32_launch: offsets must be 16-byte aligned");
-    const int64_t groups = (n[i] + 255) / 256;
-    res_off[i] = groups_total;
-    groups_total += groups;
-    tile_prefix[i + 1] = tile_prefix[i] + (groups + 31) / 32;
-  }
   const uint32_t* ex = nullptr;
   if (expect.has_value()) {
     TORCH_CHECK_VALUE(expect->is_cuda() && expect->scalar_type() == torch::kInt32 && expect->numel() >= B &&
@@ -74,27 +60,22 @@
   }
   TORCH_CHECK_VALUE(scatter_to.has_value() == scatter_idx.has_value(), "scatter_to and scatter_idx go together");
   std::vector<uint8_t> blk;
-  int64_t d_o, d_n, d_tp, d_ro, d_si = -1, d_k = -1;
-  put(blk, d_o, o, B * 8);
-  put(blk, d_n, n, B * 8);
-  put(blk, d_tp, tile_prefix.data(), (B + 1) * 8);
-  put(blk, d_ro, res_off.data(), B * 8);
   uint32_t* sout = nullptr;
   int64_t sn = 0;
+  const int64_t* sidx = nullptr;
   if (scatter_to.has_value()) {
     TORCH_CHECK_VALUE(scatter_to->is_cuda() && scatter_to->scalar_type() == torch::kInt32 && scatter_to->is_contiguous(),
                 "scatter_to: int32 GPU tensor");
-    const I64& si = *scatter_idx;
-    TORCH_CHECK_VALUE(si.size() == B, "scatter_idx size");
+    TORCH_CHECK_VALUE(scatter_idx->size() == B, "scatter_idx size");
     sn = scatter_to->numel();
-    for (int64_t i = 0; i < B; ++i) TORCH_CHECK_VALUE(si.data()[i] >= 0 && si.data()[i] < sn, "scatter index out of range");
-    put(blk, d_si, si.data(), B * 8);
+    sidx = scatter_idx->data();
     sout = static_cast<uint32_t*>(scatter_to->data_ptr());
   }
-  if (keys.has_value()) {
-    TORCH_CHECK_VALUE(keys->size() == 4 * B, "keys: int64[B, 4]");
-    put(blk, d_k, keys->data(), B * 32);
-  }
+  if (keys.has_value()) TORCH_CHECK_VALUE(keys->size() == 4 * B, "keys: int64[B, 4]");
+  const hlsp2p::host::CrcDesc d =
+      hlsp2p::host::put_crc_desc(blk, o, n, B, cap, sidx, sn, keys.has_value() ? keys->data() : nullptr);
+  const int64_t d_o = d.o, d_n = d.n, d_tp = d.tp, d_ro = d.ro, d_si = d.si, d_k = d.k;
+  const int64_t groups_total = d.groups_total;
   const int64_t nbytes = static_cast<int64_t>(blk.size());
   Tensor host = torch::empty({nbytes}, torch::TensorOptions().dtype(torch::kUInt8).pinned_memory(true));
   std::memcpy(host.data_ptr<uint8_t>(), blk.data(), blk.size());
@@ -113,7 +94,7 @@
       static_cast<const uint8_t*>(buf.data_ptr()), at(d_o), at(d_n), at(d_tp), at(d_ro), wfrag.data_ptr(),
       static_cast<const uint32_t*>(tables.data_ptr()), reinterpret_cast<uint32_t*>(base + d_res),
       reinterpret_cast<uint32_t*>(base + d_crc), ex, ex ? base + d_ok : nullptr, d_si >= 0 ? at(d_si) : nullptr, sout,
-      sn, static_cast<int>(B), tile_prefix[B], cus(device), fp4, st, d_k >= 0 ? at(d_k) : nullptr);
+      sn, static_cast<int>(B), d.total_tiles, cus(device), fp4, st, d_k >= 0 ? at(d_k) : nullptr);
   TORCH_CHECK(e == hipSuccess, "crc32 launch failed: ", hipGetErrorString(e));
   return py::make_tuple(crc, ex ? py::cast(ok) : py::none());
 }
diff --git a/hlsjs_p2p_wrapper_amd/ops/csrc/kernels/rccl_comm.cpp b/hlsjs_p2p_wrapper_amd/ops/csrc/kernels/rccl_comm.cpp
--- a/hlsjs_p2p_wrapper_amd/ops/csrc/kernels/rccl_comm.cpp
+++ b/hlsjs_p2p_wrapper_amd/ops/csrc/kernels/rccl_comm.cpp
@@ -43,18 +43,21 @@
                 py::array_t<int64_t, py::array::c_style | py::array::forcecast> recv_ptr,
                 py::array_t<int64_t, py::array::c_style | py::array::forcecast> recv_bytes,
                 py::array_t<int64_t, py::array::c_style | py::array::forcecast> recv_peer, int64_t stream) {
-    if (comm_ == nullptr) throw std::runtime_error("RcclComm: communicator is closed");
     const int64_t ns = send_ptr.size(), nr = recv_ptr.size();
     if (send_bytes.size() != ns || send_peer.size() != ns || recv_bytes.size() != nr || recv_peer.size() != nr)
       throw std::invalid_argument("RcclComm.exchange: argument sizes differ");
-    const int64_t *sp = send_ptr.data(), *sb = send_bytes.data(), *sd = send_peer.data();
-    const int64_t *rp = recv_ptr.data(), *rb = recv_bytes.data(), *rs = recv_peer.data();
+    post(send_ptr.data(), send_bytes.data(), send_peer.data(), ns, recv_ptr.data(), recv_bytes.data(),
+         recv_peer.data(), nr, reinterpret_cast<hipStream_t>(stream));
+  }
+
+  void post(const int64_t* sp, const int64_t* sb, const int64_t* sd, int64_t ns, const int64_t* rp, const int64_t* rb,
+            const int64_t* rs, int64_t nr, hipStream_t st) {
+    if (comm_ == nullptr) throw std::runtime_error("RcclComm: communicator is closed");
     for (int64_t i = 0; i < ns; ++i)
       if (sd[i] < 0 || sd[i] >= world_ || sb[i] < 0) throw std::invalid_argument("RcclComm.exchange: bad send");
     for (int64_t i = 0; i < nr; ++i)
       if (rs[i] < 0 || rs[i] >= world_ || rb[i] < 0) throw std::invalid_argument("RcclComm.exchange: bad recv");
     if (ns == 0 && nr == 0) return;
-    hipStream_t st = reinterpret_cast<hipStream_t>(stream);
     ncclResult_t r = ncclSuccess;
     {
       py::gil_scoped_release nogil;
@@ -157,6 +160,13 @@
 
 }
 
+bool rccl_post_columns(py::handle comm, const int64_t* sp, const int64_t* sb, const int64_t* sd, int64_t ns,
+                       const int64_t* rp, const int64_t* rb, const int64_t* rs, int64_t nr, hipStream_t st) {
+  if (!py::isinstance<RcclComm>(comm)) return false;
+  comm.cast<std::shared_ptr<RcclComm>>()->post(sp, sb, sd, ns, rp, rb, rs, nr, st);
+  return true;
+}
+
 void register_rccl(py::module& m) {
   m.def("rccl_unique_id", &unique_id, "ncclGetUniqueId (rank 0 of a new communicator)");
   m.def("rccl_version", &version);
diff --git a/hlsjs_p2p_wrapper_amd/ops/csrc/kernels/round_desc.h b/hlsjs_p2p_wrapper_amd/ops/csrc/kernels/round_desc.h
--- /dev/null
+++ b/hlsjs_p2p_wrapper_amd/ops/csrc/kernels/round_desc.h
@@ -0,0 +1,91 @@
+#pragma once
+
+#include <hip/hip_runtime_api.h>
+#include <torch/extension.h>
+
+#include <cstdint>
+#include <cstring>
+#include <vector>
+
+namespace hlsp2p {
+namespace host {
+
+inline int64_t issue_merged_copies(uint8_t* base, int64_t cap, const int64_t* o, const int64_t* s, const int64_t* l,
+                                   const int64_t* a, int64_t n, int64_t max_gap, bool device_src, hipStream_t st) {
+  int64_t issued = 0;
+  int64_t i = 0;
+  while (i < n) {
+    TORCH_CHECK(o[i] >= 0 && l[i] >= 0 && o[i] + l[i] <= cap, "h2d_batch: destination out of bounds");
+    if (l[i] == 0) {
+      ++i;
+      continue;
+    }
+    int64_t j = i;
+    while (j + 1 < n && l[j + 1] > 0 && a[j + 1] == a[j]) {
+      const int64_t ds = o[j + 1] - o[j], ss = s[j + 1] - s[j];
+      if (ds != ss || ds < l[j] || ds - l[j] >= max_gap) break;
+      TORCH_CHECK(o[j + 1] >= 0 && o[j + 1] + l[j + 1] <= cap, "h2d_batch: destination out of bounds");
+      ++j;
+    }
+    const int64_t bytes = o[j] + l[j] - o[i];
+    const hipError_t e =
+        hipMemcpyAsync(base + o[i], reinterpret_cast<const void*>(s[i]), static_cast<size_t>(bytes),
+                       device_src ? hipMemcpyDeviceToDevice : hipMemcpyHostToDevice, st);
+    TORCH_CHECK(e == hipSuccess, "hipMemcpyAsync launch failed: ", hipGetErrorString(e));
+    ++issued;
+    i = j + 1;
+  }
+  return issued;
+}
+
+inline void put(std::vector<uint8_t>& blk, int64_t& off, const void* p, int64_t nbytes) {
+  off = static_cast<int64_t>(blk.size());
+  blk.resize(off + ((nbytes + 15) & ~int64_t(15)), 0);
+  if (nbytes) std::memcpy(blk.data() + off, p, static_cast<size_t>(nbytes));
+}
+
+struct CrcDesc {
+  int64_t o = -1, n = -1, tp = -1, ro = -1, si = -1, k = -1;
+  int64_t groups_total = 0, total_tiles = 0;
+};
+
+inline CrcDesc put_crc_desc(std::vector<uint8_t>& blk, const int64_t* o, const int64_t* n, int64_t B, int64_t cap,
+                            const int64_t* scatter_idx, int64_t scatter_n, const int64_t* keys) {
+  CrcDesc d;
+  std::vector<int64_t> tile_prefix(B + 1, 0), res_off(B, 0);
+  for (int64_t i = 0; i < B; ++i) {
+    TORCH_CHECK_VALUE(o[i] >= 0 && n[i] >= 0 && o[i] + n[i] <= cap, "crc32_launch: range out of bounds");
+    TORCH_CHECK_VALUE(o[i] % 16 == 0, "crc32_launch: offsets must be 16-byte aligned");
+    const int64_t groups = (n[i] + 255) / 256;
+    res_off[i] = d.groups_total;
+    d.groups_total += groups;
+    tile_prefix[i + 1] = tile_prefix[i] + (groups + 31) / 32;
+  }
+  d.total_tiles = tile_prefix[B];
+  put(blk, d.o, o, B * 8);
+  put(blk, d.n, n, B * 8);
+  put(blk, d.tp, tile_prefix.data(), (B + 1) * 8);
+  put(blk, d.ro, res_off.data(), B * 8);
+  if (scatter_idx != nullptr) {
+    for (int64_t i = 0; i < B; ++i)
+      TORCH_CHECK_VALUE(scatter_idx[i] >= 0 && scatter_idx[i] < scatter_n, "scatter index out of range");
+    put(blk, d.si, scatter_idx, B * 8);
+  }
+  if (keys != nullptr) put(blk, d.k, keys, B * 32);
+  return d;
+}
+
+inline void span_columns(int64_t arena_ptr, const int64_t* runs, int64_t n, int w, int span_off, int span_len,
+                         int64_t trailer_ptr, int64_t* ptr, int64_t* nb, int64_t* peer) {
+  for (int64_t i = 0; i < n; ++i) {
+    const int64_t* r = runs + i * w;
+    ptr[2 * i] = arena_ptr + r[span_off];
+    nb[2 * i] = r[span_len];
+    ptr[2 * i + 1] = trailer_ptr + 4 * r[1];
+    nb[2 * i + 1] = 4 * (r[2] - r[1]);
+    peer[2 * i] = peer[2 * i + 1] = r[0];
+  }
+}
+
+}
+}
diff --git a/hlsjs_p2p_wrapper_amd/ops/csrc/kernels/round_post.cpp b/hlsjs_p2p_wrapper_amd/ops/csrc/kernels/round_post.cpp
--- /dev/null
+++ b/hlsjs_p2p_wrapper_amd/ops/csrc/kernels/round_post.cpp
@@ -0,0 +1,283 @@
+#include <c10/hip/HIPStream.h>
+#include <hip/hip_runtime_api.h>
+#include <torch/extension.h>
+#include <pybind11/numpy.h>
+#include <pybind11/stl.h>
+
+#include <stdexcept>
+#include <vector>
+
+#include "round_desc.h"
+
+namespace hlsp2p {
+namespace dev {
+hipError_t launch_crc32_batch(const uint8_t*, const int64_t*, const int64_t*, const int64_t*, const int64_t*,
+                              const void*, const uint32_t*, uint32_t*, uint32_t*, const uint32_t*, uint8_t*,
+                              const int64_t*, uint32_t*, int64_t, int, int64_t, int, bool, hipStream_t,
+                              const int64_t*);
+hipError_t launch_crc_table_gather(const int32_t*, int64_t, const int64_t*, int32_t*, int, hipStream_t);
+hipError_t launch_crc_table_scatter(int32_t*, int64_t, const int64_t*, const int32_t*, int, hipStream_t);
+}
+}
+
+namespace py = pybind11;
+
+bool rccl_post_columns(py::handle comm, const int64_t* sp, const int64_t* sb, const int64_t* sd, int64_t ns,
+                       const int64_t* rp, const int64_t* rb, const int64_t* rs, int64_t nr, hipStream_t st);
+
+namespace {
+
+using torch::Tensor;
+namespace H = hlsp2p::host;
+namespace D = hlsp2p::dev;
+using I64 = py::array_t<int64_t, py::array::c_style | py::array::forcecast>;
+
+int cus(int device) {
+  static int cached[64] = {0};
+  if (device >= 0 && device < 64 && cached[device]) return cached[device];
+  int n = 0;
+  hipDeviceGetAttribute(&n, hipDeviceAttributeMultiprocessorCount, device);
+  if (n <= 0) n = 256;
+  if (device >= 0 && device < 64) cached[device] = n;
+  return n;
+}
+
+void hip_ok(hipError_t e, const char* what) {
+  TORCH_CHECK(e == hipSuccess, "round_post: ", what, " failed: ", hipGetErrorString(e));
+}
+
+int64_t up256(int64_t n) { return (n + 255) / 256 * 256; }
+
+void check_table(const Tensor& t) {
+  TORCH_CHECK_VALUE(t.is_cuda() && t.scalar_type() == torch::kInt32 && t.is_contiguous() && t.dim() == 1,
+                    "crc table: contiguous 1-D int32 GPU tensor");
+}
+
+hipEvent_t order_event(int device) {
+  static hipEvent_t ev[64] = {nullptr};
+  TORCH_CHECK(device >= 0 && device < 64, "round_post: device index");
+  if (ev[device] == nullptr) hip_ok(hipEventCreateWithFlags(&ev[device], hipEventDisableTiming), "hipEventCreate");
+  return ev[device];
+}
+
+struct ExchangeFailed : std::runtime_error {
+  using std::runtime_error::runtime_error;
+};
+
+struct Columns {
+  std::vector<int64_t> sp, sb, sd, rp, rb, rs;
+};
+
+Columns build_columns(int64_t arena_ptr, const int64_t* srun, int64_t ns, int64_t send_trailers, const int64_t* rrun,
+                      int64_t nr, int64_t recv_trailers) {
+  Columns c;
+  c.sp.resize(2 * ns), c.sb.resize(2 * ns), c.sd.resize(2 * ns);
+  c.rp.resize(2 * nr), c.rb.resize(2 * nr), c.rs.resize(2 * nr);
+  H::span_columns(arena_ptr, srun, ns, 6, 4, 5, send_trailers, c.sp.data(), c.sb.data(), c.sd.data());
+  H::span_columns(arena_ptr, rrun, nr, 5, 3, 4, recv_trailers, c.rp.data(), c.rb.data(), c.rs.data());
+  return c;
+}
+
+I64 to_array(const std::vector<int64_t>& v) { return I64(static_cast<py::ssize_t>(v.size()), v.data()); }
+
+int64_t rows_of(const I64& a, int w, const char* name) {
+  if (a.size() == 0) return 0;
+  TORCH_CHECK_VALUE(a.ndim() == 2 && a.shape(1) == w, name, ": int64[n, ", w, "]");
+  return a.shape(0);
+}
+
+py::tuple round_columns(int64_t arena_ptr, I64 srun, int64_t send_trailers, I64 rrun, int64_t recv_trailers) {
+  const int64_t ns = rows_of(srun, 6, "srun"), nr = rows_of(rrun, 5, "rrun");
+  const Columns c = build_columns(arena_ptr, srun.data(), ns, send_trailers, rrun.data(), nr, recv_trailers);
+  return py::make_tuple(to_array(c.sp), to_array(c.sb), to_array(c.sd), to_array(c.rp), to_array(c.rb),
+                        to_array(c.rs));
+}
+
+void check_runs(const int64_t* runs, int64_t n, int w, int span_off, int span_len, int64_t cap, int64_t rows,
+                const char* what) {
+  for (int64_t i = 0; i < n; ++i) {
+    const int64_t* r = runs + i * w;
+    TORCH_CHECK_VALUE(r[span_off] >= 0 && r[span_len] >= 0 && r[span_off] + r[span_len] <= cap, what,
+                      ": span outside the arena");
+    TORCH_CHECK_VALUE(r[1] >= 0 && r[1] <= r[2] && r[2] <= rows, what, ": trailer slice outside its rows");
+  }
+}
+
+Tensor crc_table_gather(Tensor table, Tensor eid) {
+  check_table(table);
+  TORCH_CHECK_VALUE(eid.is_cuda() && eid.scalar_type() == torch::kInt64 && eid.is_contiguous(), "eid: int64 GPU tensor");
+  TORCH_CHECK_VALUE(eid.numel() <= INT32_MAX, "eid: too many rows");
+  Tensor out = torch::empty({eid.numel()}, table.options());
+  hipStream_t st = c10::hip::getCurrentHIPStream(table.get_device()).stream();
+  hip_ok(D::launch_crc_table_gather(static_cast<const int32_t*>(table.data_ptr()), table.numel(),
+                                    static_cast<const int64_t*>(eid.data_ptr()), static_cast<int32_t*>(out.data_ptr()),
+                                    static_cast<int>(eid.numel()), st),
+         "crc_table_gather");
+  return out;
+}
+
+void crc_table_scatter(Tensor table, Tensor rid, Tensor val) {
+  check_table(table);
+  TORCH_CHECK_VALUE(rid.is_cuda() && rid.scalar_type() == torch::kInt64 && rid.is_contiguous(), "rid: int64 GPU tensor");
+  TORCH_CHECK_VALUE(val.is_cuda() && val.scalar_type() == torch::kInt32 && val.is_contiguous() &&
+                        val.numel() == rid.numel() && rid.numel() <= INT32_MAX,
+                    "val: int32 GPU tensor, one per id");
+  hipStream_t st = c10::hip::getCurrentHIPStream(table.get_device()).stream();
+  hip_ok(D::launch_crc_table_scatter(static_cast<int32_t*>(table.data_ptr()), table.numel(),
+                                     static_cast<const int64_t*>(rid.data_ptr()),
+                                     static_cast<const int32_t*>(val.data_ptr()), static_cast<int>(rid.numel()), st),
+         "crc_table_scatter");
+}
+
+int64_t enqueue_copies(uint8_t* abase, int64_t cap, const int64_t* o, const int64_t* s, const int64_t* l,
+                       const int64_t* a, int64_t B, int64_t max_gap, bool device_src, hipStream_t cs, hipStream_t st,
+                       int64_t ev_start, int64_t ev_end, int device) {
+  if (ev_start) hip_ok(hipEventRecord(reinterpret_cast<hipEvent_t>(ev_start), cs), "hipEventRecord");
+  const int64_t dmas = H::issue_merged_copies(abase, cap, o, s, l, a, B, max_gap, device_src, cs);
+  if (ev_end) hip_ok(hipEventRecord(reinterpret_cast<hipEvent_t>(ev_end), cs), "hipEventRecord");
+  if (cs != st) {
+    hipEvent_t after = reinterpret_cast<hipEvent_t>(ev_end);
+    if (after == nullptr) {
+      after = order_event(device);
+      hip_ok(hipEventRecord(after, cs), "hipEventRecord");
+    }
+    hip_ok(hipStreamWaitEvent(st, after, 0), "hipStreamWaitEvent");
+  }
+  return dmas;
+}
+
+int64_t round_copies(Tensor arena, I64 cdn_off, I64 cdn_ptr, I64 cdn_len, I64 cdn_alloc, int64_t max_gap,
+                     bool device_src, int64_t copy_stream, int64_t ev_cdn_start, int64_t ev_cdn_end) {
+  TORCH_CHECK_VALUE(arena.is_cuda() && arena.is_contiguous() && arena.scalar_type() == torch::kUInt8 && arena.dim() == 1,
+                    "arena: contiguous 1-D GPU uint8");
+  const int64_t B = cdn_off.size();
+  TORCH_CHECK_VALUE(cdn_ptr.size() == B && cdn_len.size() == B && cdn_alloc.size() == B, "cdn columns: sizes differ");
+  if (B == 0) return 0;
+  const int device = arena.get_device();
+  hipStream_t st = c10::hip::getCurrentHIPStream(device).stream();
+  hipStream_t cs = copy_stream ? reinterpret_cast<hipStream_t>(copy_stream) : st;
+  return enqueue_copies(static_cast<uint8_t*>(arena.data_ptr()), arena.numel(), cdn_off.data(), cdn_ptr.data(),
+                        cdn_len.data(), cdn_alloc.data(), B, max_gap, device_src, cs, st, ev_cdn_start, ev_cdn_end,
+                        device);
+}
+
+py::object round_post(Tensor arena, I64 cdn_off, I64 cdn_len, bool ingest_crc, I64 cdn_eids, I64 cdn_keys,
+                      c10::optional<Tensor> wfrag, c10::optional<Tensor> tables, Tensor crc_table, I64 send_eids,
+                      I64 srun, I64 rrun, I64 recv_eids, py::object exchange, bool post_exchange, int64_t ev_p2p_start,
+                      int64_t ev_p2p_end) {
+  TORCH_CHECK_VALUE(arena.is_cuda() && arena.is_contiguous() && arena.scalar_type() == torch::kUInt8 && arena.dim() == 1,
+                    "arena: contiguous 1-D GPU uint8");
+  TORCH_CHECK_VALUE((reinterpret_cast<uintptr_t>(arena.data_ptr()) & 15) == 0, "arena must be 16-byte aligned");
+  check_table(crc_table);
+  TORCH_CHECK_VALUE(crc_table.get_device() == arena.get_device(), "crc table and arena on different devices");
+  const int device = arena.get_device();
+  const int64_t cap = arena.numel();
+  const int64_t tn = crc_table.numel();
+  uint8_t* abase = static_cast<uint8_t*>(arena.data_ptr());
+  hipStream_t st = c10::hip::getCurrentHIPStream(device).stream();
+
+  const int64_t B = cdn_off.size();
+  TORCH_CHECK_VALUE(cdn_len.size() == B, "cdn columns: sizes differ");
+  const bool crc_on = ingest_crc && B > 0;
+  bool fp4 = false;
+  if (crc_on) {
+    TORCH_CHECK_VALUE(cdn_eids.size() == B && cdn_keys.size() == 4 * B, "cdn_eids / cdn_keys: one per CDN row");
+    TORCH_CHECK_VALUE(wfrag.has_value() && tables.has_value(), "ingest_crc needs wfrag and tables");
+    fp4 = wfrag->scalar_type() == torch::kUInt8;
+    TORCH_CHECK_VALUE(wfrag->is_cuda() && wfrag->numel() >= (fp4 ? 32 * 64 * 16 : 64 * 64 * 16), "wfrag");
+    TORCH_CHECK_VALUE(tables->is_cuda() && tables->scalar_type() == torch::kInt32 && tables->numel() >= 48 * 1024,
+                      "tables");
+  }
+  const int64_t n_send = send_eids.size(), n_recv = recv_eids.size();
+  TORCH_CHECK_VALUE(n_send <= INT32_MAX && n_recv <= INT32_MAX && B <= INT32_MAX, "too many rows");
+  const int64_t ns = rows_of(srun, 6, "srun"), nr = rows_of(rrun, 5, "rrun");
+  check_runs(srun.data(), ns, 6, 4, 5, cap, n_send, "srun");
+  check_runs(rrun.data(), nr, 5, 3, 4, cap, n_recv, "rrun");
+  for (int64_t i = 0; i < ns; ++i)
+    TORCH_CHECK_VALUE(srun.data()[i * 6 + 3] == 0, "srun: a gathered run needs the general path");
+  for (int64_t i = 0; i < n_send; ++i) TORCH_CHECK_VALUE(send_eids.data()[i] < tn, "send entry id out of range");
+  for (int64_t i = 0; i < n_recv; ++i)
+    TORCH_CHECK_VALUE(recv_eids.data()[i] >= 0 && recv_eids.data()[i] < tn, "received entry id out of range");
+
+  std::vector<uint8_t> blk;
+  H::CrcDesc d;
+  if (crc_on) d = H::put_crc_desc(blk, cdn_off.data(), cdn_len.data(), B, cap, cdn_eids.data(), tn, cdn_keys.data());
+  int64_t d_se = -1, d_re = -1;
+  if (n_send) H::put(blk, d_se, send_eids.data(), n_send * 8);
+  if (n_recv) H::put(blk, d_re, recv_eids.data(), n_recv * 8);
+
+  const int64_t nbytes = static_cast<int64_t>(blk.size());
+  const int64_t d_res = up256(nbytes);
+  const int64_t d_crc = d_res + (crc_on ? up256(std::max<int64_t>(1, d.groups_total) * 4) : 0);
+  const int64_t d_st = d_crc + (crc_on ? up256(B * 4) : 0);
+  const int64_t d_rt = d_st + up256(n_send * 4);
+  const int64_t d_end = d_rt + up256(n_recv * 4);
+  Tensor dblk;
+  uint8_t* base = nullptr;
+  if (d_end > 0) {
+    dblk = torch::empty({d_end}, torch::TensorOptions().dtype(torch::kUInt8).device(torch::kCUDA, device));
+    base = dblk.data_ptr<uint8_t>();
+  }
+  if (nbytes > 0) {
+    Tensor host = torch::empty({nbytes}, torch::TensorOptions().dtype(torch::kUInt8).pinned_memory(true));
+    std::memcpy(host.data_ptr<uint8_t>(), blk.data(), blk.size());
+    dblk.narrow(0, 0, nbytes).copy_(host, true);
+  }
+  auto at = [&](int64_t off) { return reinterpret_cast<int64_t*>(base + off); };
+  int32_t* table = static_cast<int32_t*>(crc_table.data_ptr());
+  if (crc_on)
+    hip_ok(D::launch_crc32_batch(abase, at(d.o), at(d.n), at(d.tp), at(d.ro), wfrag->data_ptr(),
+                                 static_cast<const uint32_t*>(tables->data_ptr()),
+                                 reinterpret_cast<uint32_t*>(base + d_res), reinterpret_cast<uint32_t*>(base + d_crc),
+                                 nullptr, nullptr, at(d.si), reinterpret_cast<uint32_t*>(table), tn,
+                                 static_cast<int>(B), d.total_tiles, cus(device), fp4, st, at(d.k)),
+           "ingest crc32");
+  if (n_send)
+    hip_ok(D::launch_crc_table_gather(table, tn, at(d_se), reinterpret_cast<int32_t*>(base + d_st),
+                                      static_cast<int>(n_send), st),
+           "crc_table_gather");
+
+  if (post_exchange && !exchange.is_none()) {
+    const Columns c = build_columns(reinterpret_cast<int64_t>(abase), srun.data(), ns,
+                                    reinterpret_cast<int64_t>(base + d_st), rrun.data(), nr,
+                                    reinterpret_cast<int64_t>(base + d_rt));
+    if (ev_p2p_start) hip_ok(hipEventRecord(reinterpret_cast<hipEvent_t>(ev_p2p_start), st), "hipEventRecord");
+    try {
+      if (!rccl_post_columns(exchange, c.sp.data(), c.sb.data(), c.sd.data(), 2 * ns, c.rp.data(), c.rb.data(),
+                             c.rs.data(), 2 * nr, st))
+        exchange(to_array(c.sp), to_array(c.sb), to_array(c.sd), to_array(c.rp), to_array(c.rb), to_array(c.rs));
+    } catch (const std::exception& e) {
+      throw ExchangeFailed(e.what());
+    }
+    if (ev_p2p_end) hip_ok(hipEventRecord(reinterpret_cast<hipEvent_t>(ev_p2p_end), st), "hipEventRecord");
+  } else {
+    TORCH_CHECK_VALUE(ns == 0 && nr == 0, "round_post: transfers to post but no exchange");
+  }
+
+  py::object expect = py::none();
+  if (n_recv) {
+    const int32_t* tr = reinterpret_cast<const int32_t*>(base + d_rt);
+    hip_ok(D::launch_crc_table_scatter(table, tn, at(d_re), tr, static_cast<int>(n_recv), st), "crc_table_scatter");
+    Tensor eh = torch::empty({n_recv}, torch::TensorOptions().dtype(torch::kInt32).pinned_memory(true));
+    eh.copy_(dblk.narrow(0, d_rt, n_recv * 4).view(torch::kInt32), true);
+    expect = py::cast(eh);
+  }
+  return expect;
+}
+
+}
+
+void register_round_post(py::module& m) {
+  py::register_exception<ExchangeFailed>(m, "ExchangeError", PyExc_RuntimeError);
+  m.def("round_post", &round_post, py::arg("arena"), py::arg("cdn_off"), py::arg("cdn_len"), py::arg("ingest_crc"),
+        py::arg("cdn_eids"), py::arg("cdn_keys"), py::arg("wfrag"), py::arg("tables"), py::arg("crc_table"),
+        py::arg("send_eids"), py::arg("srun"), py::arg("rrun"), py::arg("recv_eids"), py::arg("exchange"),
+        py::arg("post_exchange"), py::arg("ev_p2p_start"), py::arg("ev_p2p_end"));
+  m.def("round_copies", &round_copies, py::arg("arena"), py::arg("cdn_off"), py::arg("cdn_ptr"), py::arg("cdn_len"),
+        py::arg("cdn_alloc"), py::arg("max_gap"), py::arg("device_src"), py::arg("copy_stream"),
+        py::arg("ev_cdn_start"), py::arg("ev_cdn_end"));
+  m.def("round_columns", &round_columns, py::arg("arena_ptr"), py::arg("srun"), py::arg("send_trailers"),
+        py::arg("rrun"), py::arg("recv_trailers"));
+  m.def("crc_table_gather", &crc_table_gather, py::arg("table"), py::arg("eid"));
+  m.def("crc_table_scatter", &crc_table_scatter, py::arg("table"), py::arg("rid"), py::arg("val"));
+}
diff --git a/hlsjs_p2p_wrapper_amd/ops/csrc/kernels/segment_ops.hip b/hlsjs_p2p_wrapper_amd/ops/csrc/kernels/segment_ops.hip
--- a/hlsjs_p2p_wrapper_amd/ops/csrc/kernels/segment_ops.hip
+++ b/hlsjs_p2p_wrapper_amd/ops/csrc/kernels/segment_ops.hip
@@ -42,6 +42,42 @@
   for (int64_t o = i + threadIdx.x; o < end; o += kCopyThreads) d[o] = s[o];
 }
 
+constexpr int kTableThreads = 256;
+
+__global__ __launch_bounds__(kTableThreads) void crc_table_gather_kernel(
+    const int32_t* __restrict__ table, int64_t table_n, const int64_t* __restrict__ eid, int32_t* __restrict__ out,
+    int n) {
+  const int i = blockIdx.x * kTableThreads + threadIdx.x;
+  if (i >= n) return;
+  const int64_t e = eid[i];
+  out[i] = (e >= 0 && e < table_n) ? table[e] : -1;
+}
+
+__global__ __launch_bounds__(kTableThreads) void crc_table_scatter_kernel(
+    int32_t* __restrict__ table, int64_t table_n, const int64_t* __restrict__ rid, const int32_t* __restrict__ val,
+    int n) {
+  const int i = blockIdx.x * kTableThreads + threadIdx.x;
+  if (i >= n) return;
+  const int64_t e = rid[i];
+  if (e >= 0 && e < table_n) table[e] = val[i];
+}
+
+hipError_t launch_crc_table_gather(const int32_t* table, int64_t table_n, const int64_t* eid, int32_t* out, int n,
+                                   hipStream_t stream) {
+  if (n <= 0) return hipSuccess;
+  hipLaunchKernelGGL(crc_table_gather_kernel, dim3((n + kTableThreads - 1) / kTableThreads), dim3(kTableThreads), 0,
+                     stream, table, table_n, eid, out, n);
+  return hipGetLastError();
+}
+
+hipError_t launch_crc_table_scatter(int32_t* table, int64_t table_n, const int64_t* rid, const int32_t* val, int n,
+                                    hipStream_t stream) {
+  if (n <= 0) return hipSuccess;
+  hipLaunchKernelGGL(crc_table_scatter_kernel, dim3((n + kTableThreads - 1) / kTableThreads), dim3(kTableThreads), 0,
+                     stream, table, table_n, rid, val, n);
+  return hipGetLastError();
+}
+
 hipError_t launch_segment_copy(const uint8_t* src, uint8_t* dst, const int64_t* src_off, const int64_t* dst_off,
                                const int64_t* len, const int64_t* chunk_prefix, int ncopy, int64_t total_chunks,
                                hipStream_t stream) {
diff --git a/hlsjs_p2p_wrapper_amd/parallel/comm.py b/hlsjs_p2p_wrapper_amd/parallel/comm.py
--- a/hlsjs_p2p_wrapper_amd/parallel/comm.py
+++ b/hlsjs_p2p_wrapper_amd/parallel/comm.py
@@ -316,6 +316,10 @@
         if self._rccl is None:
             return None
         return self._exchange_spans
+
+    @property
+    def rccl_native(self):
+        return self._rccl
 
     def _exchange_spans(self, sp, sb, sd, rp, rb, rs) -> None:
         if len(sp) or len(rp):
```

Measured after the change: 18920 (median of 3 runs). No clear change (+0.0%).
